# chao1224/GeoSSL

Hardware: AMD Instinct MI355X
Metric: molecules/s/GPU SchNet+DDM fwd+bwd (QM9-sized, bs=1024); % HBM roofline (higher is better)
Workload: dtype f32

## Files before the change

### geossl_amd/Geom3D/models/schnet.py

```python
import ctypes as C
import math
import os

import torch
from ...switches import env as _env
from torch.nn import Embedding, Linear, ModuleList, Sequential

from ... import _lib, ops
from ..._lib import call, ptr, stream
from ...layout import get_layout
from ._atomic_mass import atomic_masses

SUPPORTED_F = (32, 64, 128)


class _Ssp(torch.autograd.Function):
    @staticmethod
    def forward(ctx, x):
        x = x.contiguous()
        y = torch.empty_like(x)
        call("geossl_ssp_fwd", ptr(x), x.numel(), ptr(y), stream())
        ctx.save_for_backward(y)
        return y

# ... 208 lines not shown
        g_emb, g_head = grads[0], grads[1 + 9 * L:]
        g_layers = [grads[1 + 9 * l: 1 + 9 * (l + 1)] for l in range(L)]
        dh_out = dhout.contiguous()
        dyn = getattr(lay, "dyn", None)
        dN2, dP2 = (dyn.n_atoms2, dyn.n_pairs2) if dyn is not None else (None, None)
        probs = []
        daggs = [None] * L
        if cfg["chain"]:
            img = sv.get("img_bwd")
            if img is None:
                img = ops.prepare_chain([lp[k] for lp in layers for k in (4, 5, 7)] + [head[0], head[2]], transB=False)
            i_lin1, i_lin2, i_lin = img[0:3 * L:3], img[1:3 * L:3], img[2:3 * L:3]
            full = lambda: torch.empty(N, F, dtype=torch.float32, device=dev)
            du = full()
            dhs = [full() for _ in range(L + 1)]
            dys, dxs = [full() for _ in range(L)], [full() for _ in range(L)]
            daggs = [full() for _ in range(L)]

            def run_rows(a0, a1, mols, todo=None):
                rows = lambda t_: t_[a0:a1]

                def chain(x_, stages):
                    if todo is not None:
                        todo.append(("chain", x_, stages))
                    else:
                        ops.linear_chain(x_, stages, dyn_rows=dN2)

                chain(rows(dh_out), [dict(image=img[3 * L + 1], tprev=rows(sv["u"]), out=rows(du)),
                                     dict(image=img[3 * L], out=rows(dhs[L]))])
                chain(rows(dhs[L]), [dict(image=i_lin[L - 1], tprev=rows(sv["ts"][L - 1]), out=rows(dys[L - 1])),
                                     dict(image=i_lin2[L - 1], out=rows(daggs[L - 1]))])
                for l in reversed(range(L)):
                    if todo is not None:
                        todo.append(("agg", daggs[l], sv["Wf"][l], dxs[l], True))
                    else:
                        ops.aggregate(daggs[l], sv["Wf"][l], sv["pair_flag"], lay, swap=True, out=dxs[l],
                                      mols=mols)
                    stages = [dict(image=i_lin1[l], res=rows(dhs[l + 1]), out=rows(dhs[l]))]
                    if l > 0:
                        stages += [dict(image=i_lin[l - 1], tprev=rows(sv["ts"][l - 1]), out=rows(dys[l - 1])),
                                   dict(image=i_lin2[l - 1], out=rows(daggs[l - 1]))]
                    chain(rows(dxs[l]), stages)

            todo = [] if (cfg["loop"] and lay.P > 0 and 2 * L + 2 <= _lib.LOOP_MAX_OPS) else None
            if todo is not None:
                run_rows(0, N, None, todo)
                if not ops.layer_loop(todo, lay, sv["pair_flag"], N, F, stagger=cfg["loop_stagger"]):
                    todo = None
            if todo is None:
                run_rows(0, N, None)
            probs.append((dh_out, sv["u"], g_head[2], g_head[3]))
            probs.append((du, sv["h_last"], g_head[0], g_head[1]))
            for l in reversed(range(L)):
                gl = g_layers[l]
                probs.append((dhs[l + 1], sv["ts"][l], gl[7], gl[8]))
                probs.append((dys[l], sv["aggs"][l], gl[5], gl[6]))
                probs.append((dxs[l], sv["hs"][l], gl[4], None))
            dh = dhs[0]
        else:
            du = ops.linear(dh_out, head[2], transB=False, tprev=sv["u"])
            dh = ops.linear(du, head[0], transB=False)
            probs.append((dh_out, sv["u"], g_head[2], g_head[3]))
            probs.append((du, sv["h_last"], g_head[0], g_head[1]))
            pw = ops.prepare_linear([lp[k] for lp in layers for k in (4, 5, 7)], transB=False)
            for l in reversed(range(L)):
                lp, gl = layers[l], g_layers[l]
                w_lin1, w_lin2, w_lin = (pw[3 * l], pw[3 * l + 1], pw[3 * l + 2]) if pw is not None else (lp[4], lp[5], lp[7])
                dy = ops.linear(dh, w_lin, transB=False, tprev=sv["ts"][l])
                dagg = ops.linear(dy, w_lin2, transB=False)
                dx = ops.aggregate(dagg, sv["Wf"][l], sv["pair_flag"], lay, swap=True)
                dh_new = ops.linear(dx, w_lin1, transB=False, res=dh)
                probs.append((dh, sv["ts"][l], gl[7], gl[8]))
                probs.append((dy, sv["aggs"][l], gl[5], gl[6]))
                probs.append((dx, sv["hs"][l], gl[4], None))
                daggs[l] = dagg
                dh = dh_new
        P = lay.P
        fw = _lib.FilterWeights()
        gin = _lib.FilterGradIn()
        for l, lp in enumerate(layers):
            fw.w1[l], fw.b1[l], fw.w2[l], fw.b2[l] = ptr(lp[0]), ptr(lp[1]), ptr(lp[2]), ptr(lp[3])
            gin.x[l], gin.dagg[l] = ptr(sv["xs"][l]), ptr(daggs[l])
        if want_params:
            ops.linear_wgrad(probs, N, F, F, accumulate=bool(accum), dyn_rows=dN2)
            nfl = _lib.load().geossl_embedding_bwd_workspace_floats(emb_w.size(0), F)
            ws = torch.empty(nfl, dtype=torch.float32, device=dev)
            z = ctx.z
            call("geossl_embedding_bwd_dyn", ptr(z), z.stride(0) if z.numel() else 1, ptr(dh), emb_w.size(0), N, F,
                 ptr(g_emb), ptr(ws), accum, dN2, st)
            if P > 0:
                gout = _lib.FilterGradOut()
                for l, gl in enumerate(g_layers):
                    gout.dw1[l], gout.db1[l], gout.dw2[l], gout.db2[l] = ptr(gl[0]), ptr(gl[1]), ptr(gl[2]), ptr(gl[3])
                nfl = _lib.load().geossl_cfconv_filter_bwd_workspace_floats(P, L, F, G)
                ws2 = torch.empty(nfl, dtype=torch.float32, device=dev)
                call("geossl_cfconv_filter_bwd_dyn", ptr(sv["pair_d"]), ptr(sv["pair_c"]), ptr(sv["pair_flag"]),
                     ptr(lay.pair_i), ptr(lay.pair_j), P, N, C.byref(fw), C.byref(gin), L, F, G, ptr(cfg["offset"]),
                     cfg["coeff"], ptr(sv["T"]), C.byref(gout), ptr(ws2), accum, dP2, dN2, st)
            elif not direct:
                for gl in g_layers:
                    for k in range(4):
                        gl[k].zero_()
        dpos = None
        if want_pos:
            dpos = torch.zeros(N, 3, dtype=torch.float32, device=dev)
            if P > 0:
                dd = torch.empty(L, P, dtype=torch.float32, device=dev)
                call("geossl_cfconv_filter_dpos", ptr(sv["pair_d"]), ptr(sv["pair_c"]), ptr(sv["pair_flag"]),
                     ptr(lay.pair_i), ptr(lay.pair_j), P, C.byref(fw), C.byref(gin), L, F, G, ptr(cfg["offset"]),
                     cfg["coeff"], cfg["cutoff"], ptr(sv["T"]), ptr(sv["Wf"]), ptr(dd), st)
                call("geossl_pair_position_grad", ptr(ctx.pos), ptr(sv["pair_d"]), ptr(dd), ptr(lay.mol_ptr),
                     ptr(lay.pair_ptr), lay.B, P, L, ptr(dpos), st)
        if direct:
            return dpos, [None] * len(grads)
        return dpos, list(grads)


class _SchNetTapeCore(torch.autograd.Function):

    @staticmethod
    def forward(ctx, z, pos, lay, cfg, *params):
        from ... import tape as tp
        with torch.no_grad():
            x = tp.leaf(pos, bool(ctx.needs_input_grad[1]))
            ps = [tp.leaf(p, bool(n)) for p, n in zip(params, ctx.needs_input_grad[4:])]
            h = tp.schnet_atom_features(z, x, lay, cfg, ps)
        ctx.tape = (h, x, ps)
        ctx.shapes = [tuple(p.shape) for p in params]
        return h.t

    @staticmethod
    def backward(ctx, dh):
        from ... import tape as tp
        if torch.is_grad_enabled():
            raise NotImplementedError("second-order gradients (training on forces) need the fused widths: "
                                      "hidden_channels == num_filters in %s" % (SUPPORTED_F,))
        h, x, ps = ctx.tape
        wrt = [v for v in [x] + ps if v.req]
        with torch.no_grad():
            got = iter(tp.grad([h], [tp.const(dh.contiguous())], wrt))
        vals = [next(got) if v.req else None for v in [x] + ps]
        dpos = None if vals[0] is None else vals[0].t
        grads = [None if g is None else g.t.reshape(shape) for g, shape in zip(vals[1:], ctx.shapes)]
        return (None, dpos, None, None) + tuple(grads)


class _SegmentReduce(torch.autograd.Function):

    @staticmethod
    def forward(ctx, h, lay, reduce):
        ctx.lay, ctx.reduce = lay, reduce
        return ops.segment_reduce(h.contiguous(), lay, reduce)

    @staticmethod
    def backward(ctx, dout):
        return _SegmentExpand.apply(dout, ctx.lay, ctx.reduce), None, None


class _SegmentExpand(torch.autograd.Function):

    @staticmethod
    def forward(ctx, dout, lay, reduce):
        ctx.lay, ctx.reduce = lay, reduce
        dh = torch.empty(lay.N, dout.size(1), dtype=torch.float32, device=dout.device)
        call("geossl_segment_reduce_bwd", ptr(dout.contiguous()), ptr(lay.mol_ptr), lay.B, dout.size(1),
             1 if reduce == "mean" else 0, ptr(dh), 0, stream())
        return dh

    @staticmethod
    def backward(ctx, g):
        return _SegmentReduce.apply(g, ctx.lay, ctx.reduce), None, None


class SchNet(torch.nn.Module):
    def __init__(self, hidden_channels=128, num_filters=128, num_interactions=6, num_gaussians=50, cutoff=10.0,
                 node_class=None, readout="mean", dipole=False, mean=None, std=None, atomref=None):
        super().__init__()
        assert readout in ["add", "sum", "mean"]
        self.hidden_channels = hidden_channels
        self.num_filters = num_filters
        self.num_interactions = num_interactions
# ... 99 lines not shown
```

### geossl_amd/NCSN.py

```python
import ctypes as C
import os

import numpy as np
import torch
from .switches import env as _env
import torch.nn as nn
import torch.nn.functional as F

from . import _lib
from ._lib import call, ptr, stream
from .layout import get_super_edge_layout


class MultiLayerPerceptron(nn.Module):

    def __init__(self, input_dim, hidden_dims, activation="relu", dropout=0):
        super().__init__()
        self.dims = [input_dim] + hidden_dims
        self.activation = getattr(F, activation) if isinstance(activation, str) else None
        self.dropout = nn.Dropout(dropout) if dropout else None
        self.layers = nn.ModuleList()
        for i in range(len(self.dims) - 1):
            self.layers.append(nn.Linear(self.dims[i], self.dims[i + 1]))
        self.reset_parameters()
# ... 148 lines not shown
        pss = (ps[:npar], ps[npar:])
        dyn = getattr(sel, "dyn", None)
        ctx.dyn = dyn
        if dyn is not None:
            hs = (h1.detach().contiguous(),) * 2
            ctx.grad_slots = (None, None)
        else:
            hs = (h1.detach().contiguous(), h2.detach().contiguous())
            ctx.grad_slots = (getattr(h1, "_geossl_grad_slot", None), getattr(h2, "_geossl_grad_slot", None))
        heads = (_lib.NcsnHeadFwd * 2)()
        keep, saved, ws = [], [], []
        for k, (h, d, nl, dn) in enumerate(((hs[0], d1, nl1, dn1), (hs[1], d2, nl2, dn2))):
            hd = heads[k]
            d, nl, dn = d.contiguous(), nl.contiguous(), dn.contiguous()
            keep += [d, nl, dn]
            for name, p in zip(_FIELDS, pss[k]):
                setattr(hd.w, name, ptr(p))
            hd.w.sigmas = ptr(sigmas[k])
            hd.h, hd.distance, hd.noise_level, hd.distance_noise = ptr(h), ptr(d), ptr(nl), ptr(dn)
            hd.anneal_power = float(powers[k])
            loss_e = torch.empty(S, dtype=torch.float32, device=dev)
            sv = {}
            if training:
                sv = dict(a1=torch.empty(S, Fd, dtype=torch.float32, device=dev),
                          a2=torch.empty(S, Fd // 2, dtype=torch.float32, device=dev),
                          pd=torch.empty(S, dtype=torch.float32, device=dev),
                          emb=torch.empty(S, dtype=torch.float32, device=dev),
                          gscale=torch.empty(S, dtype=torch.float32, device=dev))
                for name in ("a1", "a2", "pd", "emb", "gscale"):
                    setattr(hd.saved, name, ptr(sv[name]))
            w_ = torch.empty(256, dtype=torch.float32, device=dev)
            hd.loss_e, hd.workspace = ptr(loss_e), ptr(w_)
            keep.append(loss_e)
            saved.append(sv)
            ws.append(w_)
        st = stream()
        call("geossl_ddm_loss_fwd2_dyn", C.byref(heads), ptr(sel.batch), ptr(sel.sei0), ptr(sel.sei1), S, Fd,
             None if dyn is None else dyn.n_super, None if dyn is None else dyn.n_atoms, st)
        loss = torch.empty((), dtype=torch.float32, device=dev)
        call("geossl_loss_reduce_partials2", ptr(ws[0]), ptr(ws[1]), ptr(sel.stats), float(out_scale), float(out_scale),
             ptr(loss), st)
        if training:
            ctx.sel, ctx.pss, ctx.saved, ctx.hs, ctx.sigmas = sel, pss, saved, hs, sigmas
            ctx.params, ctx.npar, ctx.out_scale = params, npar, float(out_scale)
        return loss

    @staticmethod
    def backward(ctx, gout):
        sel, pss, saved, hs = ctx.sel, ctx.pss, ctx.saved, ctx.hs
        dev = hs[0].device
        S, Fd, N = sel.S, hs[0].size(1), hs[0].size(0)
        st = stream()
        gout = gout.contiguous().to(torch.float32)
        direct = _lib.direct_grads_enabled(ctx.params)
        grads = [p.grad for p in ctx.params] if direct else [torch.empty_like(p) for p in pss[0] + pss[1]]
        gs = (grads[:ctx.npar], grads[ctx.npar:])
        lib = _lib.load()
        heads = (_lib.NcsnHeadBwd * 2)()
        keep, dhs = [], []
        nws = int(lib.geossl_ddm_loss_bwd_fused_workspace_floats(S, Fd))
        dyn = ctx.dyn
        dh_all = torch.empty(N, Fd, dtype=torch.float32, device=dev) if dyn is not None else None
        for k in range(2):
            hd = heads[k]
            for name, p in zip(_FIELDS, pss[k]):
                setattr(hd.w, name, ptr(p))
            hd.w.sigmas = ptr(ctx.sigmas[k])
            for name in ("a1", "a2", "pd", "emb", "gscale"):
                setattr(hd.saved, name, ptr(saved[k][name]))
            for name, t_ in zip(_FIELDS, gs[k]):
                setattr(hd.grads, name, ptr(t_))
            dfeat = torch.empty(S, Fd, dtype=torch.float32, device=dev)
            demb = torch.empty(S, dtype=torch.float32, device=dev)
            grow = torch.empty(S, dtype=torch.float32, device=dev)
            ws1 = torch.empty(nws, dtype=torch.float32, device=dev)
            slot = ctx.grad_slots[k]
            dh = dh_all if dyn is not None else (slot.rows(N, Fd, torch.float32, dev) if slot is not None else None)
            if dh is None:
                dh = torch.empty(N, Fd, dtype=torch.float32, device=dev)
            hd.h, hd.out_scale, hd.dfeat, hd.demb, hd.grow, hd.workspace, hd.dh = (
                ptr(hs[k]), ctx.out_scale, ptr(dfeat), ptr(demb), ptr(grow), ptr(ws1), ptr(dh))
            keep += [dfeat, demb, grow, ws1]
            dhs.append(dh)
        call("geossl_ddm_loss_bwd_fused2_dyn", C.byref(heads), ptr(sel.sei0), ptr(sel.sei1), S, sel.N if dyn is not None else N,
             Fd, ptr(sel.stats), ptr(gout), ptr(sel.inc_ptr), ptr(sel.inc_idx), 1 if direct else 0,
             None if dyn is None else dyn.n_super, None if dyn is None else dyn.n_atoms, st)
        head = ((dh_all, None) if dyn is not None else (dhs[0], dhs[1])) + (None,) * 11
        if direct:
            return head + (None,) * len(grads)
        return head + tuple(grads)


def ddm_heads_loss(n1, n2, data, h1, distance_1, h2, distance_2, noise_level_1=None, distance_noise_1=None,
                   noise_level_2=None, distance_noise_2=None, out_scale=0.5):
    ok = (isinstance(n1, NCSN_version_03) and isinstance(n2, NCSN_version_03) and n1.emb_dim == n2.emb_dim
          and n1.emb_dim in (32, 64, 128) and not _env("GEOSSL_NCSN_SPLIT_BWD")
          and not _env("GEOSSL_ARITH_24BIT")
          and not _env("GEOSSL_NCSN_SEPARATE_HEADS")
          and (h2 is None or h1.shape == h2.shape) and not distance_1.requires_grad and not distance_2.requires_grad
          and n1 is not n2 and not ({id(p) for p in _head_params(n1)} & {id(p) for p in _head_params(n2)}))
    if ok:
        S_, N_, Fd = data.super_edge_index.size(1), h1.size(0), h1.size(1)
        ok = S_ > 0 and max(S_, N_) * Fd * 4 < 2 ** 32
    bucket = getattr(data, "_bucket", None)
    if bucket is not None and (not ok or h2 is not None):
        raise _lib.GeosslHipError("a capacity-bucket batch needs the paired NCSN heads on one fused feature tensor")
    if not ok:
        return (n1(data, h1, distance_1, noise_level=noise_level_1, distance_noise=distance_noise_1, out_scale=out_scale) +
                n2(data, h2, distance_2, noise_level=noise_level_2, distance_noise=distance_noise_2, out_scale=out_scale))
    _lib.require_cuda(h1, h2, distance_1, distance_2, n1.sigmas, n2.sigmas)
    n1.device = n2.device = n1.sigmas.device
    num_graphs = data.num_graphs
    sel = bucket.sel if bucket is not None else get_super_edge_layout(data.batch, data.super_edge_index, num_graphs)
    draws = []
    for n_, nl, dn, d in ((n1, noise_level_1, distance_noise_1, distance_1), (n2, noise_level_2, distance_noise_2, distance_2)):
        if nl is None:
            nl = torch.randint(0, n_.sigmas.size(0), (num_graphs,), device=n_.sigmas.device)
        if dn is None:
            dn = torch.randn_like(d)
        draws.append((nl, dn))
    p1, p2 = _head_params(n1), _head_params(n2)
    return _NcsnLossPair.apply(h1, h2, distance_1.view(-1), distance_2.view(-1), draws[0][0], draws[0][1].view(-1),
                               draws[1][0], draws[1][1].view(-1), sel, (n1.sigmas.detach(), n2.sigmas.detach()),
                               (n1.anneal_power, n2.anneal_power), out_scale, len(p1), *p1, *p2)


class NCSN_version_03(torch.nn.Module):
    def __init__(self, emb_dim, sigma_begin, sigma_end, num_noise_level, noise_type, anneal_power):
        super().__init__()
        self.anneal_power = anneal_power
        self.noise_type = noise_type
        self.input_distance_mlp = MultiLayerPerceptron(1, [emb_dim, 1], activation="relu")
        self.output_mlp = MultiLayerPerceptron(1 + emb_dim, [emb_dim, emb_dim // 2, 1])
        sigmas = torch.tensor(np.exp(np.linspace(np.log(sigma_begin), np.log(sigma_end), num_noise_level)),
                              dtype=torch.float32)
        self.sigmas = nn.Parameter(sigmas, requires_grad=False)
        self.emb_dim = emb_dim

    def forward(self, data, node_feature, distance, debug=False, noise_level=None, distance_noise=None,
                out_scale=1.0):
        self.device = self.sigmas.device
        _lib.require_cuda(node_feature, distance, self.sigmas)
        if self.emb_dim not in (32, 64, 128):
            raise NotImplementedError("HIP path supports emb_dim in (32, 64, 128)")
        if distance.requires_grad:
            raise NotImplementedError("gradient w.r.t. distance/positions is not built (SURVEY.md §8(f) N3)")
        num_graphs = data.num_graphs
        sel = get_super_edge_layout(data.batch, data.super_edge_index, num_graphs)
        if noise_level is None:
            noise_level = torch.randint(0, self.sigmas.size(0), (num_graphs,), device=self.device)
        if distance_noise is None:
            distance_noise = torch.randn_like(distance)
        if sel.S == 0:
            raise ValueError("batch has no super edges (scatter_add over an empty index fails in the reference too)")
        loss = _NcsnLoss.apply(node_feature, distance.view(-1), noise_level, distance_noise.view(-1), sel,
                               self.sigmas.detach(), self.anneal_power, out_scale, *_head_params(self))
        if debug:
            print("loss", float(loss))
        return loss
```

### geossl_amd/_lib.py

```python
import ctypes as C
import os

import torch

HERE = os.path.dirname(os.path.abspath(__file__))
LIB_PATH = os.path.join(HERE, "lib", "libgeossl_hip.so")

MAX_L = 12
TN_MAX = 32
EPI_BIAS, EPI_SSP, EPI_RESIDUAL, EPI_MUL_DSSP, CHAIN_SAME_INPUT, CHAIN_NEW_INPUT, CHAIN_ADD_PREV = 1, 2, 4, 8, 16, 32, 64
EPI_SILU, EPI_MUL_DSILU = 128, 256

vp = C.c_void_p
i64 = C.c_int64
i32 = C.c_int
f32 = C.c_float
f64 = C.c_double
u64 = C.c_uint64


class FilterWeights(C.Structure):
    _fields_ = [("w1", vp * MAX_L), ("b1", vp * MAX_L), ("w2", vp * MAX_L), ("b2", vp * MAX_L)]


# ... 174 lines not shown
    "geossl_cfconv_filter_fwd_dyn": (i32, [vp, vp, i64, P(FilterWeights), i32, i32, i32, vp, f32, vp, vp, vp, vp]),
    "geossl_cfconv_filter_bwd_dyn": (i32, [vp, vp, vp, vp, vp, i64, i64, P(FilterWeights), P(FilterGradIn), i32, i32, i32,
                                           vp, f32, vp, P(FilterGradOut), vp, i32, vp, vp, vp]),
    "geossl_cfconv_aggregate_work_dyn": (i32, [vp, vp, vp, vp, vp, vp, i64, i32, i32, i32, vp, vp, vp]),
    "geossl_cfconv_aggregate_targets_dyn": (i32, [vp, vp, vp, vp, vp, vp, i64, i32, i32, i32, vp, vp, vp]),
    "geossl_linear_chain_dyn": (i32, [vp, i32, P(Chain), i64, i32, vp, vp]),
    "geossl_linear_wgrad_dyn": (i32, [P(TnBatch), i32, i64, i32, i32, i32, i32, i32, vp, i32, vp, vp]),
    "geossl_ddm_loss_fwd2_dyn": (i32, [vp, vp, vp, vp, i64, i32, vp, vp, vp]),
    "geossl_ddm_loss_bwd_fused2_dyn": (i32, [vp, vp, vp, i64, i64, i32, vp, vp, vp, vp, i32, vp, vp, vp]),
    "geossl_painn_group_capacity": (i64, [i64, i64]),
    "geossl_painn_edge_layout": (i32, [vp, vp, i64, vp, i64, i64, i64] + [vp] * 12),
    "geossl_painn_edge_geom_dyn": (i32, [vp, vp, vp, i64, f32, vp, vp, i32, vp, vp, vp, vp, vp]),
    "geossl_painn_interaction_fwd_mma_dyn": (i32, [vp, vp, vp, vp, vp, vp, vp, vp, vp, vp, vp, vp, vp, i64, i32, i64, i32,
                                                   i32, vp, vp, vp, vp]),
    "geossl_tape_unary": (i32, [i32, vp, i64, f32, f32, vp, vp]),
    "geossl_tape_binary": (i32, [i32, vp, i32, vp, i32, i64, i32, f32, vp, vp]),
    "geossl_tape_colsum_workspace_floats": (i64, [i64, i32]),
    "geossl_tape_reduce": (i32, [i32, vp, i64, i32, vp, vp, vp]),
    "geossl_tape_gather_rows": (i32, [vp, vp, i32, i64, i32, vp, vp]),
    "geossl_tape_scatter_rows": (i32, [vp, vp, i32, vp, i64, i32, vp, vp]),
    "geossl_tape_copy2d": (i32, [vp, i64, vp, i64, i64, i32, vp]),
    "geossl_tape_fill": (i32, [vp, i64, f32, vp]),
    "geossl_painn_stage_cap": (i32, [i32, i32, i32]),
    "geossl_painn_interaction_fwd_atoms": (i32, [vp] * 12 + [i64, vp, i32, i32, vp, vp, vp]),
    "geossl_painn_interaction_bwd_atoms": (i32, [vp] * 13 + [i64, vp, i32, i32, vp, vp, vp, vp, vp, i32, vp]),
    "geossl_painn_interaction_bwd_mol_skip": (i32, [vp, vp, vp, vp, vp, vp, vp, vp, vp, vp, vp, vp, vp, i64, i32, i64, i32,
                                                    i32, vp, vp, vp, vp, vp, i32, vp]),
    "geossl_painn_mix_pre_fwd_dyn": (i32, [vp, vp, i64, i32, f32, vp, vp, vp, vp]),
    "geossl_painn_mix_post_fwd_dyn": (i32, [vp, vp, vp, vp, vp, i64, i32, vp, vp, vp, vp]),
    "geossl_painn_mix_post_bwd_dyn": (i32, [vp, vp, vp, vp, vp, i64, i32, vp, vp, vp, vp]),
    "geossl_painn_mix_pre_bwd_dyn": (i32, [vp, vp, vp, vp, i64, i32, vp, vp, vp, vp]),
    "geossl_gather_molecules": (i32, [P(Gather), i64, vp]),
    "geossl_gather_masked_molecules": (i32, [P(Gather), P(Mask), i64, vp]),
    "geossl_infonce_fwd": (i32, [vp, vp, i64, i32, f32, vp, vp, vp, vp, vp]),
    "geossl_infonce_bwd": (i32, [vp, vp, vp, vp, i64, i32, f32, vp, vp, vp, vp]),
    "geossl_ebm_nce_fwd": (i32, [vp, vp, i64, i32, i32, vp, vp, vp, vp, vp, vp]),
    "geossl_ebm_nce_bwd": (i32, [vp, vp, vp, i64, i32, i32, vp, vp, vp, vp]),
    "geossl_distance_head_width_ok": (i32, [i32]),
    "geossl_distance_head_fwd_workspace_floats": (i64, [i64]),
    "geossl_distance_head_bwd_workspace_floats": (i64, [i64, i32]),
    "geossl_distance_head_fwd": (i32, [vp, i64, i32, vp, vp, vp, vp, vp, i64, vp, vp, vp, vp, vp, vp]),
    "geossl_distance_head_fwd_dyn": (i32, [vp, i64, i32, vp, vp, vp, vp, vp, i64, vp, vp, vp, vp, vp, vp, vp, vp]),
    "geossl_distance_head_bwd": (i32, [vp, i64, i32, vp, vp, i64, vp, vp, vp, vp, vp, vp, vp, vp, i32, vp]),
    "geossl_distance_head_bwd_dyn": (i32, [vp, i64, i32, vp, vp, i64, vp, vp, vp, vp, vp, vp, vp, vp, i32, vp, vp, vp]),
    "geossl_charge_mask_count": (i64, [i64, f64]),
    "geossl_charge_mask": (i32, [vp, i32, i64, f64, i32, vp, vp, vp, vp, vp, vp]),
    "geossl_charge_mask_dyn": (i32, [vp, i32, i64, f64, i32, vp, vp, vp, vp, vp, vp, vp]),
    "geossl_charge_head_width_ok": (i32, [i32, i32]),
    "geossl_charge_head_fwd_workspace_floats": (i64, [i64]),
    "geossl_charge_head_bwd_workspace_floats": (i64, [i64, i32, i32]),
    "geossl_charge_head_fwd": (i32, [vp, i64, i32, vp, vp, i32, vp, vp, i64, vp, vp, vp, vp, vp, vp]),
    "geossl_charge_head_fwd_dyn": (i32, [vp, i64, i32, vp, vp, i32, vp, vp, i64, vp, vp, vp, vp, vp, vp, vp]),
    "geossl_charge_head_bwd": (i32, [vp, i64, i32, vp, i32, vp, vp, i64, vp, vp, vp, vp, vp, vp, vp, i32, vp]),
    "geossl_charge_head_bwd_dyn": (i32, [vp, i64, i32, vp, i32, vp, vp, i64, vp, vp, vp, vp, vp, vp, vp, i32, vp, vp]),
    "geossl_infograph_width_ok": (i32, [i32]),
    "geossl_infograph_fwd_workspace_floats": (i64, [i64]),
    "geossl_infograph_fwd": (i32, [vp, i64, i32, vp, vp, i64, i32, vp, vp, vp, vp, vp, vp, vp, vp]),
    "geossl_infograph_fwd_dyn": (i32, [vp, i64, i32, vp, vp, i64, i32, vp, vp, vp, vp, vp, vp, vp, vp, vp]),
    "geossl_infograph_bwd": (i32, [vp, i64, i32, vp, vp, i64, i32, vp, vp, vp, vp, vp, vp, vp, vp]),
    "geossl_infograph_bwd_dyn": (i32, [vp, i64, i32, vp, vp, i64, i32, vp, vp, vp, vp, vp, vp, vp, vp, vp]),
    "geossl_property_width_ok": (i32, [i32]),
    "geossl_property_workspace_floats": (i64, [i64]),
    "geossl_property_fwd": (i32, [vp, i64, i32, vp, i64, i32, i32, vp, vp, vp, vp, vp, i64, vp, i32, vp, vp, vp, vp, vp,
                                  vp]),
    "geossl_property_fwd_dyn": (i32, [vp, i64, i32, vp, i64, i32, i32, vp, vp, vp, vp, vp, i64, vp, i32, vp, vp, vp, vp,
                                      vp, vp, vp]),
    "geossl_property_predict": (i32, [vp, i64, i32, vp, i64, i32, i32, vp, vp, vp, vp, vp, vp, vp]),
    "geossl_property_predict_dyn": (i32, [vp, i64, i32, vp, i64, i32, i32, vp, vp, vp, vp, vp, vp, vp, vp]),
    "geossl_property_bwd": (i32, [i64, i32, vp, i64, i32, i32, vp, vp, vp, vp, vp, vp, i64, vp, i32, vp, vp, vp, vp, vp,
                                  vp, i32, vp]),
    "geossl_property_bwd_dyn": (i32, [i64, i32, vp, i64, i32, i32, vp, vp, vp, vp, vp, vp, i64, vp, i32, vp, vp, vp, vp,
                                      vp, vp, i32, vp, vp]),
    "geossl_property_targets": (i32, [vp, i64, i32, i32, vp, vp, i64, vp, vp]),
    "geossl_torsion_head_width_ok": (i32, [i32]),
    "geossl_torsion_head_fwd_workspace_floats": (i64, [i64]),
    "geossl_torsion_head_bwd_workspace_floats": (i64, [i64, i32]),
    "geossl_torsion_head_fwd": (i32, [vp, i64, i32, vp, vp, vp, vp, vp, vp, i64, vp, vp, vp, vp, vp, vp]),
    "geossl_torsion_head_fwd_dyn": (i32, [vp, i64, i32, vp, vp, vp, vp, vp, vp, i64, vp, vp, vp, vp, vp, vp, vp, vp]),
    "geossl_torsion_head_bwd": (i32, [vp, i64, i32, vp, vp, vp, vp, i64, vp, vp, i64, vp, vp, vp, vp, vp, i32, vp]),
    "geossl_torsion_head_bwd_dyn": (i32, [vp, i64, i32, vp, vp, vp, vp, i64, vp, vp, i64, vp, vp, vp, vp, vp, i32, vp, vp,
                                          vp]),
    "geossl_triple_angles": (i32, [vp, i64, vp, vp, vp, i64, vp, vp]),
    "geossl_gather_triples": (i32, [vp, i64, vp, vp, vp, vp, i64, vp, vp, vp, vp, vp]),
}

_lib = None


class GeosslHipError(RuntimeError):
    pass


def load():
    global _lib
    if _lib is not None:
        return _lib
    path = os.environ.get("GEOSSL_HIP_LIB", LIB_PATH)
    if not os.path.exists(path):
        raise GeosslHipError(
            "libgeossl_hip.so is not built (%s). Run `python -m geossl_amd.build` (needs hipcc); "
            "there is no CPU fallback." % path)
    lib = C.CDLL(path)
    for name, (res, args) in PROTOTYPES.items():
        fn = getattr(lib, name)
        fn.restype = res
        fn.argtypes = args
    if lib.geossl_abi_version() != 1:
        raise GeosslHipError("ABI version mismatch")
    _lib = lib
    return lib


def check(rc, what):
    if rc != 0:
        raise GeosslHipError("%s failed with hipError %d" % (what, rc))


def ptr(t):
    if t is None:
        return None
    return t.data_ptr()


def stream():
    return torch._C._cuda_getCurrentRawStream(torch._C._cuda_getDevice())


def require_cuda(*tensors):
    for t in tensors:
        if t is not None and not t.is_cuda:
            raise GeosslHipError(
                "geossl_amd runs on MI355X only: got a %s tensor. The HIP path has no CPU fallback." % t.device.type)



_DIRECT = {"depth": 0}


class direct_grads:
    def __enter__(self):
        _DIRECT["depth"] += 1
        return self

    def __exit__(self, *exc):
        _DIRECT["depth"] -= 1
        return False


def direct_grads_enabled(params):
    return _DIRECT["depth"] > 0 and all(
        p.grad is not None and p.grad.is_contiguous() and p.grad.dtype == torch.float32 and p.grad.is_cuda
        for p in params)


class StatusWord:

    def __init__(self, device, message):
        self.word = torch.zeros(1, dtype=torch.int32, device=device)
        self.host = torch.zeros(1, dtype=torch.int32).pin_memory()
        self.event = None
        self.message = message

    def __deepcopy__(self, memo):
        return None

    def __reduce__(self):
        return (type(None), ())

    def poll(self):
        if self.event is None or torch.cuda.is_current_stream_capturing():
            return
        if self.event.query():
            self.event = None
            if int(self.host[0]):
                raise IndexError(self.message)

    def arm(self, every=1):
        self.calls = getattr(self, "calls", 0) + 1
        if every > 1 and self.calls % every != 1:
            return
        if self.event is None and not torch.cuda.is_current_stream_capturing():
            self.host.copy_(self.word, non_blocking=True)
            self.event = torch.cuda.Event()
            self.event.record()

    def check(self):
        if int(self.word.item()):
            raise IndexError(self.message)


def module_status(module, device, message):
    st = module.__dict__.get("_geossl_status")
    if st is None or st.word.device != device:
        st = StatusWord(device, message)
        module.__dict__["_geossl_status"] = st
    return st


TIMERS = None
CALLS = None


def call(name, *args):
    global CALLS
    lib = load()
    if CALLS is not None:
        CALLS += 1
    timers = TIMERS
    key = name[:-4] if name.endswith("_dyn") else name
    if timers is not None and key in timers:
        e0, e1 = torch.cuda.Event(enable_timing=True), torch.cuda.Event(enable_timing=True)
        e0.record()
        rc = getattr(lib, name)(*args)
        e1.record()
        timers[key].append((e0, e1))
    else:
        rc = getattr(lib, name)(*args)
    check(rc, name)


def fill_ptrs(arr, tensors):
    for i, t in enumerate(tensors):
        arr[i] = ptr(t)
```

### geossl_amd/build.py

```python
import os
import subprocess
import sys

HERE = os.path.dirname(os.path.abspath(__file__))
REPO = os.path.dirname(HERE)
CSRC = os.path.join(HERE, "csrc")
LIB_DIR = os.path.join(HERE, "lib")
LIB_PATH = os.path.join(LIB_DIR, "libgeossl_hip.so")


def _sources():
    return sorted(f for f in os.listdir(CSRC) if f.endswith(".hip"))


SOURCE_FLAGS = {"painn_mma.hip": ["-fno-slp-vectorize"], "distance_head.hip": ["-fno-slp-vectorize"],
                "charge_head.hip": ["-fno-slp-vectorize"], "infograph_head.hip": ["-fno-slp-vectorize"],
                "property_head.hip": ["-fno-slp-vectorize"], "torsion_head.hip": ["-fno-slp-vectorize"]}


def _headers():
    hs = [os.path.join(CSRC, f) for f in os.listdir(CSRC) if f.endswith(".h")]
    inc = os.path.join(REPO, "include")
    return hs + [os.path.join(inc, f) for f in os.listdir(inc) if f.endswith(".h")]


def source_hash():
    import hashlib
    h = hashlib.sha256()
    h.update(repr(sorted(SOURCE_FLAGS.items())).encode())
    for path in sorted([os.path.join(CSRC, s_) for s_ in _sources()] + _headers()):
        h.update(os.path.basename(path).encode() + b"\0")
        with open(path, "rb") as fh:
            h.update(fh.read())
    return h.hexdigest()[:16]


def _newest(paths):
    return max(os.path.getmtime(p) for p in paths)


def needs_build():
    if not os.path.exists(LIB_PATH):
        return True
    deps = [os.path.join(CSRC, s) for s in _sources()] + _headers() + [os.path.abspath(__file__)]
    return _newest(deps) > os.path.getmtime(LIB_PATH)


def build(force=False, verbose=True):
    if not force and not needs_build():
        return LIB_PATH
    os.makedirs(LIB_DIR, exist_ok=True)
    hipcc = os.environ.get("HIPCC", "/opt/rocm/bin/hipcc")
    objs = []
    procs = []
    for s in _sources():
        obj = os.path.join(LIB_DIR, s.replace(".hip", ".o"))
        cmd = [hipcc, "--offload-arch=gfx950", "-O3", "-std=c++17", "-fPIC", "-I", os.path.join(REPO, "include"),
               "-I", CSRC, "-Wno-pass-failed"] + SOURCE_FLAGS.get(s, []) + ["-c", os.path.join(CSRC, s), "-o", obj]
        if verbose:
            print(" ".join(cmd), flush=True)
        procs.append((cmd, subprocess.Popen(cmd)))
        objs.append(obj)
    for cmd, p in procs:
        if p.wait() != 0:
            raise RuntimeError("hipcc failed: " + " ".join(cmd))
    cmd = [hipcc, "--offload-arch=gfx950", "-shared", "-fPIC", "-o", LIB_PATH] + objs
    if verbose:
        print(" ".join(cmd), flush=True)
    subprocess.check_call(cmd)
    return LIB_PATH


if __name__ == "__main__":
    build(force="--force" in sys.argv)
    print(LIB_PATH)
```

### geossl_amd/csrc/common.h

```cpp
#pragma once
#include <hip/hip_runtime.h>
#include <stdint.h>

#include <mutex>

typedef float f32x16 __attribute__((ext_vector_type(16)));
typedef float f32x4 __attribute__((ext_vector_type(4)));

#define GEOSSL_MAX_LAYERS 12
#define GEOSSL_PI_F 3.14159265358979323846f

#define GEOSSL_CHECK_LAUNCH()                  \
  do {                                         \
    hipError_t e__ = hipGetLastError();        \
    if (e__ != hipSuccess) return (int)e__;    \
  } while (0)

namespace geossl {

inline void allow_big_lds_ptr(const void* kernel) {
  struct Seen { const void* fn; int dev; };
  static Seen seen[512];
  static int nseen = 0;
  static std::mutex mu;
// ... 21 lines not shown
#pragma clang fp contract(off)
  const float xx = x * x, yy = y * y, zz = z * z;
  return (xx + yy) + zz;
}

__device__ __forceinline__ void lds_barrier() {
  asm volatile("s_waitcnt lgkmcnt(0)\n\ts_barrier" ::: "memory");
}

__device__ __forceinline__ float wave_max(float v) {
  v = fmaxf(v, __builtin_bit_cast(float, __builtin_amdgcn_update_dpp(0, __builtin_bit_cast(int, v), 0xB1, 0xF, 0xF, false)));
  v = fmaxf(v, __builtin_bit_cast(float, __builtin_amdgcn_update_dpp(0, __builtin_bit_cast(int, v), 0x4E, 0xF, 0xF, false)));
  v = fmaxf(v, __builtin_bit_cast(float, __builtin_amdgcn_update_dpp(0, __builtin_bit_cast(int, v), 0x141, 0xF, 0xF, false)));
  v = fmaxf(v, __builtin_bit_cast(float, __builtin_amdgcn_update_dpp(0, __builtin_bit_cast(int, v), 0x140, 0xF, 0xF, false)));
  const float a = __builtin_bit_cast(float, __builtin_amdgcn_readlane(__builtin_bit_cast(int, v), 0));
  const float b = __builtin_bit_cast(float, __builtin_amdgcn_readlane(__builtin_bit_cast(int, v), 16));
  const float c = __builtin_bit_cast(float, __builtin_amdgcn_readlane(__builtin_bit_cast(int, v), 32));
  const float d = __builtin_bit_cast(float, __builtin_amdgcn_readlane(__builtin_bit_cast(int, v), 48));
  return fmaxf(fmaxf(a, b), fmaxf(c, d));
}
__device__ __forceinline__ int wave_max_i32(int v) {
  v = max(v, __builtin_amdgcn_update_dpp(v, v, 0xB1, 0xF, 0xF, false));
  v = max(v, __builtin_amdgcn_update_dpp(v, v, 0x4E, 0xF, 0xF, false));
  v = max(v, __builtin_amdgcn_update_dpp(v, v, 0x141, 0xF, 0xF, false));
  v = max(v, __builtin_amdgcn_update_dpp(v, v, 0x140, 0xF, 0xF, false));
  return max(max(__builtin_amdgcn_readlane(v, 0), __builtin_amdgcn_readlane(v, 16)),
             max(__builtin_amdgcn_readlane(v, 32), __builtin_amdgcn_readlane(v, 48)));
}
__device__ __forceinline__ int c_row(int reg, int lane) { return (reg & 3) + 8 * (reg >> 2) + 4 * (lane >> 5); }

#define GEOSSL_SSP_SHIFT 0.693147182464599609375f
__device__ __forceinline__ float exp_neg(float x) { return __builtin_amdgcn_exp2f(x * 1.44269504088896340736f); }
__device__ __forceinline__ float ssp(float x) {
  const float z = exp_neg(-fabsf(x));
  const float l = __builtin_amdgcn_logf(1.0f + z);
  return fmaf(l, 0.693147180559945309417f, fmaxf(x, 0.0f)) - GEOSSL_SSP_SHIFT;
}
__device__ __forceinline__ float dssp_from_out(float t) { return 1.0f - 0.5f * exp_neg(-t); }

template <class ValFn, class ConsumeFn>
__device__ __forceinline__ void transpose_c_block(float* stage, int lane, ValFn val, ConsumeFn consume) {
  const int j = lane & 31, kh = lane >> 5;
  const int rr = lane >> 3, c4 = lane & 7;
#pragma unroll
  for (int half = 0; half < 2; ++half) {
#pragma unroll
    for (int q = 0; q < 8; ++q) {
      const int r = 8 * half + q;
      const int row16 = (r & 3) + 8 * ((r >> 2) & 1) + 4 * kh;
      stage[row16 * 32 + j] = val(r);
    }
    asm volatile("s_waitcnt lgkmcnt(0)" ::: "memory");
#pragma unroll
    for (int u = 0; u < 2; ++u) {
      const int row16 = 8 * u + rr;
      const float4 v = *reinterpret_cast<const float4*>(stage + row16 * 32 + 4 * c4);
      consume(16 * half + row16, 4 * c4, v);
    }
    asm volatile("s_waitcnt lgkmcnt(0)" ::: "memory");
  }
}

__device__ __forceinline__ float pin(float v) {
  asm volatile("" : "+v"(v));
  return v;
}
__device__ __forceinline__ float4 pin(float4 v) {
  asm volatile("" : "+v"(v.x), "+v"(v.y), "+v"(v.z), "+v"(v.w));
  return v;
}

__device__ __forceinline__ float kahan_sum_strided(const float* __restrict__ p, int b0, int b1, int stride) {
#pragma clang fp reassociate(off) contract(off)
  float s = 0.0f, c = 0.0f;
#pragma unroll 4
  for (int b = b0; b < b1; ++b) {
    const float y = p[(size_t)b * stride] - c;
    const float t = s + y;
    c = (t - s) - y;
    s = t;
  }
  return s;
}

__device__ __forceinline__ int dyn_count(int cap, const int32_t* __restrict__ dyn) {
  return dyn != nullptr ? min(cap, *dyn) : cap;
}

__device__ __forceinline__ float wave_sum(float v) {
#pragma unroll
  for (int o = 32; o > 0; o >>= 1) v += __shfl_xor(v, o, 64);
  return v;
}

}
```

### geossl_amd/csrc/filter_bwd.hip

```cpp
#include "common.h"
#include "geossl_hip.h"
#include "split.h"
#include "tn.h"

using namespace geossl;

namespace {

#ifdef FB_TIMING
__device__ long long fb_dbg[2 * 64 * 8];
__device__ long long fb_dbg2[2 * 64];
__device__ long long fb_dbg3[64 * 4];
#define FB_MARK(slot)                                                                                   \
  do {                                                                                                  \
    if (blockIdx.x == 3 && blockIdx.y == 0 && lane == 0 && (wave == 0 || wave == NW) && t - t_begin < 64) \
      fb_dbg[((wave == 0 ? 0 : 1) * 64 + (t - t_begin)) * 8 + (slot)] = clock64();                      \
  } while (0)
#define FB3(slot)                                                                                      \
  do {                                                                                                  \
    __builtin_amdgcn_sched_barrier(0);                                                                  \
    if (blockIdx.x == 3 && blockIdx.y == 0 && lane == 0 && wave == NW && tt - t_begin < 64 && tt > t_begin) \
      fb_dbg3[(tt - t_begin) * 4 + (slot)] = clock64();                                                  \
    __builtin_amdgcn_sched_barrier(0);                                                                  \
  } while (0)
// ... 1043 lines not shown

}

#ifdef FB_TIMING
extern "C" int geossl_filter_bwd_debug_read(long long* host) {
  return (int)hipMemcpyFromSymbol(host, HIP_SYMBOL(fb_dbg), sizeof(long long) * 2 * 64 * 8);
}
extern "C" int geossl_filter_bwd_debug_read3(long long* host) {
  return (int)hipMemcpyFromSymbol(host, HIP_SYMBOL(fb_dbg3), sizeof(long long) * 64 * 4);
}
extern "C" int geossl_filter_bwd_debug_read2(long long* host) {
  return (int)hipMemcpyFromSymbol(host, HIP_SYMBOL(fb_dbg2), sizeof(long long) * 2 * 64);
}
#endif

extern "C" int64_t geossl_cfconv_filter_bwd_workspace_floats(int64_t P, int L, int F, int G) {
  const int ntiles = (int)((P + TR - 1) / TR);
  const int64_t nb = blocks_per_layer(L, ntiles);
  return (int64_t)L * nb * ((int64_t)F * G + F + (int64_t)F * F + F);
}

extern "C" int geossl_cfconv_filter_bwd(const float* pair_d, const float* pair_c, const uint8_t* pair_flag,
                                        const int32_t* pair_i, const int32_t* pair_j, int64_t P, int64_t N,
                                        const GeosslFilterWeights* w, const GeosslFilterGradIn* g, int L, int F, int G,
                                        const float* offset, float coeff, const float* T,
                                        const GeosslFilterGradOut* out, float* workspace, int accumulate,
                                        hipStream_t stream) {
  return geossl_cfconv_filter_bwd_dyn(pair_d, pair_c, pair_flag, pair_i, pair_j, P, N, w, g, L, F, G, offset, coeff, T, out,
                                      workspace, accumulate, nullptr, nullptr, stream);
}

extern "C" int geossl_cfconv_filter_bwd_dyn(const float* pair_d, const float* pair_c, const uint8_t* pair_flag,
                                            const int32_t* pair_i, const int32_t* pair_j, int64_t P, int64_t N,
                                            const GeosslFilterWeights* w, const GeosslFilterGradIn* g, int L, int F,
                                            int G, const float* offset, float coeff, const float* T,
                                            const GeosslFilterGradOut* out, float* workspace, int accumulate,
                                            const int32_t* dyn_P, const int32_t* dyn_N, hipStream_t stream) {
  if (P <= 0 || L <= 0) return 0;
  if (L > GEOSSL_MAX_L || (F != 32 && F != 64 && F != 128) || G > 64) return (int)hipErrorInvalidValue;
  const int ntiles = (int)((P + TR - 1) / TR);
  const int nb = blocks_per_layer(L, ntiles);
  dim3 grid(nb, L);
  float* pw1 = workspace;
  float* pb1 = pw1 + (size_t)L * nb * F * G;
  float* pw2 = pb1 + (size_t)L * nb * F;
  float* pb2 = pw2 + (size_t)L * nb * F * F;
#define LAUNCH(NW)                                                                                                 \
  do {                                                                                                             \
    const size_t lds = BwdLds<32 * NW>::bytes();                                                                   \
    allow_big_lds(&k_filter_bwd<NW>);                                                                              \
    hipLaunchKernelGGL((k_filter_bwd<NW>), grid, dim3(128 * NW), lds, stream, pair_d, pair_c, pair_flag, pair_i,   \
                       pair_j, (int)P, (int)N, *w, *g, G, offset, coeff, T, pw1, pb1, pw2, pb2, dyn_P, dyn_N);     \
  } while (0)
#define LAUNCH_H(NW)                                                                                               \
  do {                                                                                                             \
    const size_t lds = BwdLdsH<32 * NW>::bytes();                                                                  \
    if (T == nullptr) {                                                                                            \
      allow_big_lds(&k_filter_bwd_h<NW, true>);                                                                    \
      hipLaunchKernelGGL((k_filter_bwd_h<NW, true>), grid, dim3(128 * NW), lds, stream, pair_d, pair_c, pair_flag, \
                         pair_i, pair_j, (int)P, (int)N, *w, *g, G, offset, coeff, T, pw1, pb1, pw2, pb2, dyn_P,   \
                         dyn_N);                                                                                   \
    } else {                                                                                                       \
      allow_big_lds(&k_filter_bwd_h<NW, false>);                                                                   \
      hipLaunchKernelGGL((k_filter_bwd_h<NW, false>), grid, dim3(128 * NW), lds, stream, pair_d, pair_c, pair_flag,\
                         pair_i, pair_j, (int)P, (int)N, *w, *g, G, offset, coeff, T, pw1, pb1, pw2, pb2, dyn_P,   \
                         dyn_N);                                                                                   \
    }                                                                                                              \
  } while (0)
  const bool bf16x3 = getenv("GEOSSL_FILTER_BWD_BF16X3") != nullptr || getenv("GEOSSL_ARITH_24BIT") != nullptr;
  if (bf16x3 && T == nullptr) return (int)hipErrorInvalidValue;
  if (!bf16x3) {
    if (F == 128) LAUNCH_H(4); else if (F == 64) LAUNCH_H(2); else LAUNCH_H(1);
  } else {
    if (F == 128) LAUNCH(4); else if (F == 64) LAUNCH(2); else LAUNCH(1);
  }
#undef LAUNCH_H
#undef LAUNCH
  GEOSSL_CHECK_LAUNCH();
  ReduceMulti rm;
  rm.add(pw1, F * G, G, G, 1, out->dw1, L);
  rm.add(pb1, F, F, F, 1, out->db1, L);
  rm.add(pw2, F * F, F, F, 1, out->dw2, L);
  rm.add(pb2, F, F, F, 1, out->db2, L);
  hipLaunchKernelGGL(k_reduce_multi, dim3(rm.blocks(), L), dim3(256), 0, stream, rm, nb, accumulate);
  GEOSSL_CHECK_LAUNCH();
  return 0;
}
```

### geossl_amd/csrc/ncsn_bwd.hip

```cpp
#include "common.h"
#include "geossl_hip.h"
#include "split.h"
#include "tn.h"

using namespace geossl;

namespace {

constexpr int TR = 32;

#ifdef NB_TIMING
__device__ long long nb_dbg[2 * 32 * 8];
#define NB_MARK(slot)                                                                              \
  do {                                                                                             \
    if (blockIdx.x == 5 && lane == 0 && (wave == 0 || wave == NW) && t - t_begin < 32)             \
      nb_dbg[((wave == 0 ? 0 : 1) * 32 + (t - t_begin)) * 8 + (slot)] = clock64();                 \
  } while (0)
#else
#define NB_MARK(slot) do {} while (0)
#endif

template <int NW>
struct NbLds {
  static constexpr int F = 32 * NW, H = F / 2, KHS = (H + 15) / 16, HMB = (H + 31) / 32, KS = F / 16;
  u32x4* zb;
  u32x4* dz2T;
  u32x4* fT;
  u32x4* dz1r;
  u32x4* abT;
  int4* scal;
  float* pdv;
  float* dep;
  float* wls;
  int* eg;
  int* ef;
  int* ea;
  int* ec;
  __device__ explicit NbLds(uint8_t* smem) {
    zb = reinterpret_cast<u32x4*>(smem);
    dz2T = zb + 2 * KHS * 2 * 64;
    fT = dz2T + HMB * 2 * 2 * 64;
    dz1r = fT + 2 * NW * 2 * 2 * 64;
    abT = dz1r + KS * 2 * 64;
    scal = reinterpret_cast<int4*>(abT + NW * 2 * 2 * 64);
    pdv = reinterpret_cast<float*>(scal + 3 * TR);
    dep = pdv + 3 * TR;
    wls = dep + NW * TR;
    eg = reinterpret_cast<int*>(wls + F);
    ef = eg + 4;
    ea = ef + 2 * NW;
    ec = ea + NW;
  }
  static size_t bytes() {
    return (size_t)(2 * KHS * 2 + HMB * 4 + 2 * NW * 4 + KS * 2 + NW * 4) * 1024 + 3 * TR * sizeof(int4) +
           (size_t)(3 * TR + NW * TR + F) * sizeof(float) + (size_t)(4 + 4 * NW) * sizeof(int);
  }
};

struct NcsnFusedArgs {
  const float* h;
  const int64_t* sei0;
  const int64_t* sei1;
  int S;
  GeosslNcsnWeights w;
  GeosslNcsnSaved sv;
  const int64_t* divisor;
  float out_scale;
  const float* gout;
  float* dfeat;
  float* demb;
  float* grow;
  float* pw1;
  float* pd1;
  float* pb1;
  float* pw2;
  float* pb2;
  float* psm;
};

__device__ __forceinline__ float ldg_off(const float* base, uint32_t byte_off) {
  return *reinterpret_cast<const float*>(reinterpret_cast<const char*>(base) + byte_off);
}
__device__ __forceinline__ int crow4(int r, int k4) { return (r & 3) + 8 * (r >> 2) + k4; }
__device__ __forceinline__ int opaque(int v) {
  asm volatile("" : "+v"(v));
  return v;
// ... 473 lines not shown
    }
    NB_MARK(4);
  }
  const size_t pb = blockIdx.x;
  if constexpr (ROLE_A) {
    float* P1 = a.pw1 + pb * F * F;
#pragma unroll
    for (int kb = 0; kb < NW; ++kb) {
      const float f = pow2(max(E1[kb] + eC - 28, -200));
#pragma unroll
      for (int r = 0; r < 16; ++r) P1[(size_t)(32 * nb + c_row(r, lane)) * F + 32 * kb + j] = accw1[kb][r] * f;
    }
    const float sb = bsum + __shfl_xor(bsum, 32, 64), sd = dsum + __shfl_xor(dsum, 32, 64);
    if (kh == 0) {
      a.pb1[pb * F + col] = sb;
      a.pd1[pb * F + col] = sd;
    }
    float* Ps = a.psm + pb * (H + 3 * F + 2);
    const float t_w2 = s_w2 + __shfl_xor(s_w2, 32, 64);
    const float t_w1 = s_w1 + __shfl_xor(s_w1, 32, 64), t_b1 = s_b1 + __shfl_xor(s_b1, 32, 64);
    if (kh == 0) {
      Ps[H + col] = t_w2;
      Ps[H + F + col] = t_w1;
      Ps[H + 2 * F + col] = t_b1;
    }
    if (wave == 0) {
      const float tg = wave_sum(s_g), td = wave_sum(s_d);
      if (lane == 0) {
        Ps[H + 3 * F] = tg;
        Ps[H + 3 * F + 1] = td;
      }
    }
  } else {
    float* P2 = a.pw2 + pb * H * F;
    const float f = pow2(max(E2 + e3 - 28, -200));
#pragma unroll
    for (int mb = 0; mb < HMB; ++mb)
#pragma unroll
      for (int r = 0; r < 16; ++r) {
        const int m = 32 * mb + c_row(r, lane);
        if (m < H) P2[(size_t)m * F + col] = accw2[mb][r] * f;
      }
    const float sb = bsum + __shfl_xor(bsum, 32, 64);
    if (nb < HMB && kh == 0 && (int)col < H) a.pb2[pb * H + col] = sb;
    if (nb < KHS) {
      float* Ps = a.psm + pb * (H + 3 * F + 2);
#pragma unroll
      for (int e = 0; e < 8; ++e) {
        float v = o3acc[e];
#pragma unroll
        for (int o = 16; o > 0; o >>= 1) v += __shfl_xor(v, o, 64);
        const int m = 16 * nb + 8 * kh + e;
        if (j == 0 && m < H) Ps[m] = v;
      }
    }
  }
}

template <int NW>
__global__ __launch_bounds__(128 * NW) void k_ncsn_bwd_fused(NcsnFusedArgs a) {
  if ((int)(threadIdx.x >> 6) < NW) ncsn_bwd_body<NW, true>(a, a.S, a.h);
  else ncsn_bwd_body<NW, false>(a, a.S, a.h);
}
struct NcsnFusedPair { NcsnFusedArgs a[2]; };
template <int NW>
__global__ __launch_bounds__(128 * NW) void k_ncsn_bwd_fused2(NcsnFusedPair pr, const int32_t* __restrict__ dyn_S,
                                                              const int32_t* __restrict__ dyn_view) {
  const NcsnFusedArgs& a = pr.a[blockIdx.y];
  const int S = dyn_count(a.S, dyn_S);
  const float* h = a.h;
  if (dyn_view != nullptr && blockIdx.y == 1) h += (size_t)(*dyn_view) * (32 * NW);
  if ((int)(threadIdx.x >> 6) < NW) ncsn_bwd_body<NW, true>(a, S, h);
  else ncsn_bwd_body<NW, false>(a, S, h);
}

__device__ __forceinline__ void ncsn_reduce_all_block(const ReduceMulti& m, int nblk, int accumulate,
                                                      const float* __restrict__ psm, int F, const GeosslNcsnGrads& g,
                                                      float (*red)[64]) {
  const int mb = m.xoff[m.nseg];
  if ((int)blockIdx.x < mb) {
    reduce_multi_block(m, nblk, accumulate, red, 0);
    return;
  }
  const int H = F / 2, len = H + 3 * F + 2;
  const int i = ((int)blockIdx.x - mb) * 4 + (int)(threadIdx.x >> 6), lane = threadIdx.x & 63;
  if (i >= len) return;
  float s = 0.0f;
  for (int b = lane; b < nblk; b += 64) s += psm[(size_t)b * len + i];
  s = wave_sum(s);
  if (lane == 0) {
    float* dst;
    if (i < H) dst = g.o3_w + i;
    else if (i < H + F) dst = g.in_w2 + (i - H);
    else if (i < H + 2 * F) dst = g.in_w1 + (i - H - F);
    else if (i < H + 3 * F) dst = g.in_b1 + (i - H - 2 * F);
    else if (i == H + 3 * F) dst = g.o3_b;
    else dst = g.in_b2;
    *dst = accumulate ? *dst + s : s;
  }
}
__global__ __launch_bounds__(256) void k_ncsn_reduce_all(ReduceMulti m, int nblk, int accumulate,
                                                         const float* __restrict__ psm, int F, GeosslNcsnGrads g) {
  __shared__ float red[4][64];
  ncsn_reduce_all_block(m, nblk, accumulate, psm, F, g, red);
}
__global__ __launch_bounds__(256) void k_ncsn_reduce_all2(ReduceMulti m0, ReduceMulti m1, int nblk, int accumulate,
                                                          const float* __restrict__ psm0,
                                                          const float* __restrict__ psm1, int F, GeosslNcsnGrads g0,
                                                          GeosslNcsnGrads g1) {
  __shared__ float red[4][64];
  if (blockIdx.y == 0) ncsn_reduce_all_block(m0, nblk, accumulate, psm0, F, g0, red);
  else ncsn_reduce_all_block(m1, nblk, accumulate, psm1, F, g1, red);
}

inline int fused_blocks(int64_t S) {
  const int64_t ntiles = (S + TR - 1) / TR;
  return (int)(ntiles < 256 ? ntiles : 256);
}

}

#ifdef NB_TIMING
extern "C" int geossl_ncsn_bwd_debug_read(long long* host) {
  return (int)hipMemcpyFromSymbol(host, HIP_SYMBOL(nb_dbg), sizeof(long long) * 2 * 32 * 8);
}
#endif

extern "C" int64_t geossl_ddm_loss_bwd_fused_workspace_floats(int64_t S, int F) {
  const int64_t nb = fused_blocks(S), H = F / 2;
  return nb * ((int64_t)F * F + 2 * F + H * F + H + (H + 3 * F + 2));
}

extern "C" int geossl_ddm_loss_bwd_fused(const float* h, const int64_t* sei0, const int64_t* sei1, int64_t S, int64_t N,
                                         int F, const GeosslNcsnWeights* w, const GeosslNcsnSaved* saved,
                                         const int64_t* stats_divisor, float out_scale, const float* gout, float* dfeat,
                                         float* demb, float* grow, const GeosslNcsnGrads* grads, float* workspace,
                                         int accumulate, hipStream_t stream) {
  if (S <= 0) return 0;
  if (F != 32 && F != 64 && F != 128) return (int)hipErrorInvalidValue;
  if (S * (int64_t)F * 4 >= ((int64_t)1 << 32) || N * (int64_t)F * 4 >= ((int64_t)1 << 32)) return (int)hipErrorInvalidValue;
  const int nb = fused_blocks(S), H = F / 2;
  NcsnFusedArgs a;
  a.h = h; a.sei0 = sei0; a.sei1 = sei1; a.S = (int)S; a.w = *w; a.sv = *saved; a.divisor = stats_divisor;
  a.out_scale = out_scale; a.gout = gout; a.dfeat = dfeat; a.demb = demb; a.grow = grow;
  a.pw1 = workspace;
  a.pd1 = a.pw1 + (size_t)nb * F * F;
  a.pb1 = a.pd1 + (size_t)nb * F;
  a.pw2 = a.pb1 + (size_t)nb * F;
  a.pb2 = a.pw2 + (size_t)nb * H * F;
  a.psm = a.pb2 + (size_t)nb * H;
#define LAUNCH(NWV)                                                                                      \
  do {                                                                                                   \
    allow_big_lds(&k_ncsn_bwd_fused<NWV>);                                                               \
    hipLaunchKernelGGL((k_ncsn_bwd_fused<NWV>), dim3(nb), dim3(128 * NWV), NbLds<NWV>::bytes(), stream, a); \
  } while (0)
  if (F == 128) LAUNCH(4); else if (F == 64) LAUNCH(2); else LAUNCH(1);
#undef LAUNCH
  GEOSSL_CHECK_LAUNCH();
  ReduceMulti rm;
  float* o1w[1] = {grads->o1_w};
  float* o1c[1] = {grads->o1_w + F};
  float* o1b[1] = {grads->o1_b};
  float* o2w[1] = {grads->o2_w};
  float* o2b[1] = {grads->o2_b};
  rm.add(a.pw1, F * F, F, F + 1, 1, o1w, 1);
  rm.add(a.pd1, F, F, F, F + 1, o1c, 1);
  rm.add(a.pb1, F, F, F, 1, o1b, 1);
  rm.add(a.pw2, H * F, F, F, 1, o2w, 1);
  rm.add(a.pb2, H, H, H, 1, o2b, 1);
  hipLaunchKernelGGL(k_ncsn_reduce_all, dim3(rm.blocks() + (H + 3 * F + 2 + 3) / 4, 1), dim3(256), 0, stream, rm, nb,
                     accumulate, a.psm, F, *grads);
  GEOSSL_CHECK_LAUNCH();
  return 0;
}

namespace geossl {
int launch_incidence_gather2(const float* dfeat0, const float* dfeat1, const int64_t* inc_ptr, const int32_t* inc_idx,
                             int64_t N, int F, float* dh0, float* dh1, hipStream_t stream, const int32_t* dyn_view);
}

extern "C" int geossl_ddm_loss_bwd_fused2(const GeosslNcsnHeadBwd* heads, const int64_t* sei0, const int64_t* sei1,
                                          int64_t S, int64_t N, int F, const int64_t* stats_divisor, const float* gout,
                                          const int64_t* inc_ptr, const int32_t* inc_idx, int accumulate,
                                          hipStream_t stream) {
  return geossl_ddm_loss_bwd_fused2_dyn(heads, sei0, sei1, S, N, F, stats_divisor, gout, inc_ptr, inc_idx, accumulate,
                                        nullptr, nullptr, stream);
}

extern "C" int geossl_ddm_loss_bwd_fused2_dyn(const GeosslNcsnHeadBwd* heads, const int64_t* sei0, const int64_t* sei1,
                                              int64_t S, int64_t N, int F, const int64_t* stats_divisor,
                                              const float* gout, const int64_t* inc_ptr, const int32_t* inc_idx,
                                              int accumulate, const int32_t* dyn_S, const int32_t* dyn_view,
                                              hipStream_t stream) {
  if (S <= 0) return 0;
  if (heads == nullptr || (F != 32 && F != 64 && F != 128)) return (int)hipErrorInvalidValue;
  if (S * (int64_t)F * 4 >= ((int64_t)1 << 32) || N * (int64_t)F * 4 >= ((int64_t)1 << 32)) return (int)hipErrorInvalidValue;
  const int nb = (fused_blocks(S) + 1) / 2, H = F / 2;
  NcsnFusedPair pr;
  NcsnFusedArgs* a = pr.a;
  for (int k = 0; k < 2; ++k) {
    const GeosslNcsnHeadBwd& hd = heads[k];
    if (hd.h == nullptr || hd.dfeat == nullptr || hd.workspace == nullptr) return (int)hipErrorInvalidValue;
    NcsnFusedArgs& x = a[k];
    x.h = hd.h; x.sei0 = sei0; x.sei1 = sei1; x.S = (int)S; x.w = hd.w; x.sv = hd.saved; x.divisor = stats_divisor;
    x.out_scale = hd.out_scale; x.gout = gout; x.dfeat = hd.dfeat; x.demb = hd.demb; x.grow = hd.grow;
    x.pw1 = hd.workspace;
    x.pd1 = x.pw1 + (size_t)nb * F * F;
    x.pb1 = x.pd1 + (size_t)nb * F;
    x.pw2 = x.pb1 + (size_t)nb * F;
    x.pb2 = x.pw2 + (size_t)nb * H * F;
    x.psm = x.pb2 + (size_t)nb * H;
  }
#define LAUNCH2(NWV)                                                                                                \
  do {                                                                                                              \
    allow_big_lds(&k_ncsn_bwd_fused2<NWV>);                                                                         \
    hipLaunchKernelGGL((k_ncsn_bwd_fused2<NWV>), dim3(nb, 2), dim3(128 * NWV), NbLds<NWV>::bytes(), stream, pr,         \
                       dyn_S, dyn_view);                                                                            \
  } while (0)
  if (F == 128) LAUNCH2(4); else if (F == 64) LAUNCH2(2); else LAUNCH2(1);
#undef LAUNCH2
  GEOSSL_CHECK_LAUNCH();
  ReduceMulti rm[2];
  for (int k = 0; k < 2; ++k) {
    const GeosslNcsnGrads* grads = &heads[k].grads;
    float* o1w[1] = {grads->o1_w};
    float* o1c[1] = {grads->o1_w + F};
    float* o1b[1] = {grads->o1_b};
    float* o2w[1] = {grads->o2_w};
    float* o2b[1] = {grads->o2_b};
    rm[k].add(a[k].pw1, F * F, F, F + 1, 1, o1w, 1);
    rm[k].add(a[k].pd1, F, F, F, F + 1, o1c, 1);
    rm[k].add(a[k].pb1, F, F, F, 1, o1b, 1);
    rm[k].add(a[k].pw2, H * F, F, F, 1, o2w, 1);
    rm[k].add(a[k].pb2, H, H, H, 1, o2b, 1);
  }
  hipLaunchKernelGGL(k_ncsn_reduce_all2, dim3(rm[0].blocks() + (H + 3 * F + 2 + 3) / 4, 2), dim3(256), 0, stream, rm[0],
                     rm[1], nb, accumulate, a[0].psm, a[1].psm, F, heads[0].grads, heads[1].grads);
  GEOSSL_CHECK_LAUNCH();
  if (heads[0].dh != nullptr && heads[1].dh != nullptr)
    return launch_incidence_gather2(heads[0].dfeat, heads[1].dfeat, inc_ptr, inc_idx, N, F, heads[0].dh, heads[1].dh, stream,
                                    dyn_view);
  return 0;
}
```

### geossl_amd/csrc/schnet.hip

```cpp
#include "common.h"
#include "aggregate_reg.h"
#include "geossl_hip.h"
#include "tn.h"

#include <cstdlib>

using namespace geossl;

namespace {

inline int grid1d(int64_t n, int block, int cap = 2048) {
  int64_t g = (n + block - 1) / block;
  return (int)(g < 1 ? 1 : (g > cap ? cap : g));
}

__global__ void k_rbf(const float* __restrict__ d, int64_t E, const float* __restrict__ offset, int G, float coeff,
                      float* __restrict__ out) {
  for (int64_t i = (int64_t)blockIdx.x * blockDim.x + threadIdx.x; i < E * G; i += (int64_t)gridDim.x * blockDim.x) {
    const int64_t e = i / G;
    const int g = (int)(i - e * G);
    const float diff = d[e] - offset[g];
    out[i] = expf(coeff * (diff * diff));
  }
}

__global__ void k_ssp_fwd(const float* __restrict__ x, int64_t n, float* __restrict__ y) {
  for (int64_t i = (int64_t)blockIdx.x * blockDim.x + threadIdx.x; i < n; i += (int64_t)gridDim.x * blockDim.x)
    y[i] = ssp(x[i]);
}
__global__ void k_ssp_bwd(const float* __restrict__ y, const float* __restrict__ dy, int64_t n, float* __restrict__ dx) {
  for (int64_t i = (int64_t)blockIdx.x * blockDim.x + threadIdx.x; i < n; i += (int64_t)gridDim.x * blockDim.x)
    dx[i] = dy[i] * dssp_from_out(y[i]);
}

__global__ void k_pair_product(const float* __restrict__ a, const float* __restrict__ b,
                               const int32_t* __restrict__ pair_i, const int32_t* __restrict__ pair_j,
                               const uint8_t* __restrict__ pair_flag, int64_t P, int F, int swap,
                               float* __restrict__ out) {
  const int Q = F / 4;
  for (int64_t idx = (int64_t)blockIdx.x * blockDim.x + threadIdx.x; idx < P * Q; idx += (int64_t)gridDim.x * blockDim.x) {
    const int64_t p = idx / Q;
    const int c = 4 * (int)(idx - p * Q);
    unsigned fl = pair_flag[p];
    if (swap) fl = ((fl & 1u) << 1) | ((fl >> 1) & 1u);
    const float f0 = (fl & 1u) ? 1.0f : 0.0f, f1 = (fl & 2u) ? 1.0f : 0.0f;
    const size_t oi = (size_t)pair_i[p] * F + c, oj = (size_t)pair_j[p] * F + c;
    const f32x4 ai = *reinterpret_cast<const f32x4*>(a + oi), aj = *reinterpret_cast<const f32x4*>(a + oj);
    const f32x4 bi = *reinterpret_cast<const f32x4*>(b + oi), bj = *reinterpret_cast<const f32x4*>(b + oj);
    *reinterpret_cast<f32x4*>(out + (size_t)p * F + c) = f0 * (ai * bj) + f1 * (aj * bi);
  }
}


template <int VW>
struct AggVec;
template <>
struct AggVec<1> {
  typedef float type;
};
template <>
struct AggVec<2> {
  typedef f32x2 type;
};

template <int VW>
__global__ __launch_bounds__(64) void k_aggregate(const float* __restrict__ x, const float* __restrict__ Wf,
                                                  const uint8_t* __restrict__ pair_flag,
                                                  const int32_t* __restrict__ mol_ptr,
                                                  const int32_t* __restrict__ pair_ptr,
                                                  const int32_t* __restrict__ order, int B, int F, int max_n, int swap,
                                                  float* __restrict__ out) {
#pragma clang fp contract(off)
  typedef typename AggVec<VW>::type V;
  extern __shared__ __attribute__((aligned(16))) float smem[];
  if ((int)blockIdx.x >= B) return;
  const int m = order != nullptr ? order[blockIdx.x] : (int)blockIdx.x;
  const int lane = threadIdx.x, f = VW * lane;
  const bool col = f < F;
  const int a0 = mol_ptr[m], n = mol_ptr[m + 1] - a0, base = pair_ptr[m], np = n * (n - 1) / 2;
  float* xs = smem;
  float* acc = smem + max_n * F;
  uint8_t* sfl = reinterpret_cast<uint8_t*>(smem + 2 * max_n * F);
  for (int p = lane; p < np; p += 64) {
    unsigned fl = pair_flag[base + p];
    if (swap) fl = ((fl & 1u) << 1) | ((fl >> 1) & 1u);
    sfl[p] = (uint8_t)fl;
// ... 136 lines not shown
      else if (part == 2) AGG_PART(4, 2); else AGG_PART(4, 3);
    }
  }
#undef AGG_PART
}

__device__ __forceinline__ int work_item(const int32_t* __restrict__ work, int nwork, const int32_t* __restrict__ dyn_nwork) {
  const int nw = dyn_count(nwork, dyn_nwork), b = (int)blockIdx.x;
  if (b >= nw) return -1;
  return work[(b & 7) * (nw >> 3) + (b >> 3)];
}

__global__ __launch_bounds__(64, 2) void k_aggregate_reg_work(
    const float* __restrict__ x, const float* __restrict__ Wf, const uint8_t* __restrict__ pair_flag,
    const int32_t* __restrict__ mol_ptr, const int32_t* __restrict__ pair_ptr, const int32_t* __restrict__ work,
    int nwork, int F, int swap, float* __restrict__ out, const int32_t* __restrict__ dyn_nwork) {
  const int wk = work_item(work, nwork, dyn_nwork);
  if (wk == -1) return;
  const int m = wk & 0x00FFFFFF, part = __builtin_amdgcn_readfirstlane((wk >> 24) & 255);
  const int lane = threadIdx.x, f = 2 * lane < F ? 2 * lane : -2;
  const int a0 = mol_ptr[m], n = mol_ptr[m + 1] - a0, base = pair_ptr[m];
  const int nu = __builtin_amdgcn_readfirstlane(n);
  if (nu > 33) {
    aggregate_targets(x, Wf, pair_flag, a0, n, base, lane, f, F, swap, out, part, part + 1);
    return;
  }
  const int kparts = nu < AGG_K2_MIN ? 1 : (nu < AGG_K4_MIN ? 2 : 4);
#define AGG_CLASS(NM) if (nu <= NM) { aggregate_reg_body<NM>(x, Wf, pair_flag, a0, n, base, lane, f, F, swap, out); return; }
#define AGG_CLASS_BIG(NM) if (nu <= NM) { aggregate_big<NM>(x, Wf, pair_flag, a0, n, base, lane, f, F, swap, out, kparts, part); return; }
  AGG_CLASS(8) AGG_CLASS(12) AGG_CLASS(16) AGG_CLASS(18) AGG_CLASS(20)
  AGG_CLASS_BIG(22) AGG_CLASS_BIG(24) AGG_CLASS_BIG(26) AGG_CLASS_BIG(28) AGG_CLASS_BIG(30) AGG_CLASS_BIG(33)
#undef AGG_CLASS
#undef AGG_CLASS_BIG
}

__global__ __launch_bounds__(64, 2) void k_aggregate_targets(
    const float* __restrict__ x, const float* __restrict__ Wf, const uint8_t* __restrict__ pair_flag,
    const int32_t* __restrict__ mol_ptr, const int32_t* __restrict__ pair_ptr, const int32_t* __restrict__ work,
    int nwork, int F, int swap, float* __restrict__ out, const int32_t* __restrict__ dyn_nwork) {
  const int wk = work_item(work, nwork, dyn_nwork);
  if (wk == -1) return;
  const int m = wk & 0x00FFFFFF, a = __builtin_amdgcn_readfirstlane((wk >> 24) & 255);
  const int lane = threadIdx.x, f = 2 * lane < F ? 2 * lane : -2;
  const int a0 = mol_ptr[m], n = mol_ptr[m + 1] - a0, base = pair_ptr[m];
  aggregate_targets(x, Wf, pair_flag, a0, n, base, lane, f, F, swap, out, a, a + 1);
}

__global__ void k_embedding_fwd(const int64_t* __restrict__ z, int64_t zs, const float* __restrict__ table, int C,
                                int64_t N, int F, float* __restrict__ out, int32_t* __restrict__ status,
                                const int32_t* __restrict__ dyn_N) {
  N = dyn_count((int)N, dyn_N);
  for (int64_t i = (int64_t)blockIdx.x * blockDim.x + threadIdx.x; i < N * F; i += (int64_t)gridDim.x * blockDim.x) {
    const int64_t a = i / F;
    const int f = (int)(i - a * F);
    const int64_t c = z[a * zs];
    if (c < 0 || c >= C) {
      if (status != nullptr) *status = 1;
      out[i] = 0.0f;
    } else {
      out[i] = table[c * F + f];
    }
  }
}
template <int SH4>
__global__ __launch_bounds__(256) void k_embedding_fwd4(const int64_t* __restrict__ z, int64_t zs,
                                                        const float* __restrict__ table, int C, int N,
                                                        float* __restrict__ out, int32_t* __restrict__ status,
                                                        const int32_t* __restrict__ dyn_N) {
  N = dyn_count(N, dyn_N);
  const uint32_t total = (uint32_t)N << SH4;
  for (uint32_t i = blockIdx.x * 256u + threadIdx.x; i < total; i += gridDim.x * 256u) {
    const uint32_t a = i >> SH4, f4 = i & ((1u << SH4) - 1u);
    const int64_t c = z[(int64_t)a * zs];
    f32x4 v = {0.0f, 0.0f, 0.0f, 0.0f};
    if (c < 0 || c >= C) {
      if (status != nullptr) *status = 1;
    } else {
      v = reinterpret_cast<const f32x4*>(table)[((uint32_t)c << SH4) + f4];
    }
    reinterpret_cast<f32x4*>(out)[i] = v;
  }
}

#define GEOSSL_EMB_CHUNKS 512
template <int NG>
__global__ void k_embedding_bwd_partial(const int64_t* __restrict__ z, int64_t zs, const float* __restrict__ dh,
                                        int64_t N, int F, int C, float* __restrict__ partial, int2* __restrict__ band,
                                        const int32_t* __restrict__ dyn_N) {
  extern __shared__ __attribute__((aligned(16))) float smem[];
  N = dyn_count((int)N, dyn_N);
  const int TF = blockDim.x / NG;
  const int chunk = blockIdx.x, grp = threadIdx.x / TF, f = threadIdx.x - grp * TF;
  const int64_t per = (N + (int64_t)gridDim.x - 1) / (int64_t)gridDim.x;
  const int64_t lo = chunk * per, hi = min((int64_t)N, lo + per);
  float* tab = smem + (size_t)grp * C * F;
  int2* gband = reinterpret_cast<int2*>(smem + (size_t)NG * C * F);
  int cmin = C, cmax = -1;
  if (f < F) {
    for (int c = 0; c < C; ++c) tab[c * F + f] = 0.0f;
    constexpr int U = 16;
    for (int64_t a0 = lo + grp; a0 < hi; a0 += (int64_t)U * NG) {
      float v[U];
      int cls[U];
#pragma unroll
      for (int u = 0; u < U; ++u) {
        const int64_t a = min(a0 + (int64_t)u * NG, hi - 1);
        v[u] = dh[a * F + f];
        cls[u] = (int)z[a * zs];
      }
#pragma unroll
      for (int u = 0; u < U; ++u)
        if (a0 + (int64_t)u * NG < hi && cls[u] >= 0 && cls[u] < C) {
          tab[cls[u] * F + f] += v[u];
          cmin = min(cmin, cls[u]);
          cmax = max(cmax, cls[u]);
        }
    }
    if (f == 0) gband[grp] = make_int2(cmin, cmax);
  }
  if (NG > 1) {
    __syncthreads();
    if (grp != 0) return;
    for (int g = 0; g < NG; ++g) {
      cmin = min(cmin, gband[g].x);
      cmax = max(cmax, gband[g].y);
    }
  }
  if (f >= F) return;
  for (int c = cmin; c <= cmax; ++c) {
    float sum = smem[c * F + f];
    for (int g = 1; g < NG; ++g) sum += smem[((size_t)g * C + c) * F + f];
    partial[((size_t)chunk * C + c) * F + f] = sum;
  }
  if (f == 0) band[chunk] = make_int2(cmin, cmax);
}
__global__ __launch_bounds__(256) void k_embedding_bwd_reduce(const float* __restrict__ partial,
                                                              const int2* __restrict__ band, int nchunks, int C, int F,
                                                              float* __restrict__ dtable, int accumulate) {
  constexpr int PERMAX = GEOSSL_EMB_CHUNKS / 4;
  static_assert(PERMAX == 128, "two chunks per lane");
  const int PER = nchunks / 4;
  __shared__ float red[4][64];
  __shared__ int hits[4][PERMAX];
  const int c = blockIdx.y, lane = threadIdx.x & 63, slice = threadIdx.x >> 6;
  const int f = blockIdx.x * 64 + lane;
  int n = 0;
#pragma unroll
  for (int h = 0; h < 2; ++h) {
    const int b = slice * PER + 64 * h + lane;
    const int2 r = 64 * h + lane < PER ? band[b] : make_int2(1, 0);
    const bool hit = c >= r.x && c <= r.y;
    const unsigned long long m = __ballot(hit);
    if (hit) hits[slice][n + __popcll(m & ((1ull << lane) - 1ull))] = b;
    n += __popcll(m);
  }
  __builtin_amdgcn_wave_barrier();
  float s = 0.0f;
  if (f < F) {
#pragma clang fp reassociate(off) contract(off)
    float k = 0.0f;
    const float* p = partial + (size_t)c * F + f;
#pragma unroll 4
    for (int i = 0; i < n; ++i) {
      const float y = p[(size_t)hits[slice][i] * C * F] - k;
      const float t = s + y;
      k = (t - s) - y;
      s = t;
    }
  }
  red[slice][lane] = s;
  __syncthreads();
  if (slice == 0 && f < F) {
    float v = accumulate ? dtable[(size_t)c * F + f] : 0.0f;
    v += red[0][lane];
    v += red[1][lane];
    v += red[2][lane];
    v += red[3][lane];
    dtable[(size_t)c * F + f] = v;
  }
}
__global__ void k_segment_reduce_fwd(const float* __restrict__ h, const int32_t* __restrict__ mol_ptr, int B, int F,
                                     int mean, float* __restrict__ out) {
  const int m = blockIdx.x;
  if (m >= B) return;
  const int a0 = mol_ptr[m], a1 = mol_ptr[m + 1];
  for (int f = threadIdx.x; f < F; f += blockDim.x) {
    float s = 0.0f;
    for (int a = a0; a < a1; ++a) s += h[(size_t)a * F + f];
    if (mean) s = s / fmaxf((float)(a1 - a0), 1.0f);
    out[(size_t)m * F + f] = s;
  }
}
__global__ void k_segment_reduce_bwd(const float* __restrict__ dout, const int32_t* __restrict__ mol_ptr, int B, int F,
                                     int mean, float* __restrict__ dh, int accumulate) {
  const int m = blockIdx.x;
  if (m >= B) return;
  const int a0 = mol_ptr[m], a1 = mol_ptr[m + 1];
  const float cnt = fmaxf((float)(a1 - a0), 1.0f);
  for (int f = threadIdx.x; f < F; f += blockDim.x) {
    float gv = dout[(size_t)m * F + f];
    if (mean) gv = gv / cnt;
    for (int a = a0; a < a1; ++a) {
      const size_t o = (size_t)a * F + f;
      dh[o] = accumulate ? dh[o] + gv : gv;
    }
  }
}

__global__ __launch_bounds__(256) void k_row_normalize_fwd(const float* __restrict__ h, int64_t N, int F, float eps,
                                                           float* __restrict__ y, float* __restrict__ norm) {
  const int lane = threadIdx.x & 63;
  const int64_t row = (int64_t)blockIdx.x * 4 + (threadIdx.x >> 6);
  if (row >= N) return;
  const float* hr = h + row * F;
  float ss = 0.0f;
  for (int f = lane; f < F; f += 64) ss = fmaf(hr[f], hr[f], ss);
  ss = wave_sum(ss);
  const float nr = sqrtf(ss), den = fmaxf(nr, eps);
  for (int f = lane; f < F; f += 64) y[row * F + f] = hr[f] / den;
  if (lane == 0 && norm != nullptr) norm[row] = nr;
}
__global__ __launch_bounds__(256) void k_row_normalize_bwd(const float* __restrict__ g, const float* __restrict__ y,
                                                           const float* __restrict__ norm, int64_t N, int F, float eps,
                                                           float* __restrict__ dh) {
  const int lane = threadIdx.x & 63;
  const int64_t row = (int64_t)blockIdx.x * 4 + (threadIdx.x >> 6);
  if (row >= N) return;
  const float* gr = g + row * F;
  const float* yr = y + row * F;
  float dot = 0.0f;
  for (int f = lane; f < F; f += 64) dot = fmaf(gr[f], yr[f], dot);
  dot = wave_sum(dot);
  const float nr = norm[row];
  const bool clamped = nr < eps;
  const float inv = 1.0f / fmaxf(nr, eps);
  for (int f = lane; f < F; f += 64) dh[row * F + f] = (clamped ? gr[f] : gr[f] - yr[f] * dot) * inv;
}

inline int blocks_per_layer(int L, int ntiles) {
  int b = 256 / (L > 0 ? L : 1);
  if (b < 1) b = 1;
  if (b > ntiles) b = ntiles;
  return b;
}

}

extern "C" int geossl_rbf_fwd(const float* d, int64_t E, const float* offset, int G, float coeff, float* out,
                              hipStream_t stream) {
  if (E <= 0) return 0;
  hipLaunchKernelGGL(k_rbf, dim3(grid1d(E * G, 256)), dim3(256), 0, stream, d, E, offset, G, coeff, out);
  GEOSSL_CHECK_LAUNCH();
  return 0;
}

extern "C" int geossl_ssp_fwd(const float* x, int64_t n, float* y, hipStream_t stream) {
  if (n <= 0) return 0;
  hipLaunchKernelGGL(k_ssp_fwd, dim3(grid1d(n, 256)), dim3(256), 0, stream, x, n, y);
  GEOSSL_CHECK_LAUNCH();
  return 0;
}
extern "C" int geossl_ssp_bwd(const float* y, const float* dy, int64_t n, float* dx, hipStream_t stream) {
// ... 77 lines not shown
    allow_big_lds(&k_aggregate<2>);
    hipLaunchKernelGGL(k_aggregate<2>, dim3((unsigned)B), dim3(64), lds, stream, x, Wf, pair_flag, mol_ptr, pair_ptr,
                       order, (int)B, F, max_n, swap, out);
  } else {
    allow_big_lds(&k_aggregate<1>);
    hipLaunchKernelGGL(k_aggregate<1>, dim3((unsigned)B), dim3(64), lds, stream, x, Wf, pair_flag, mol_ptr, pair_ptr,
                       order, (int)B, F, max_n, swap, out);
  }
  GEOSSL_CHECK_LAUNCH();
  return 0;
}

extern "C" int geossl_row_normalize_fwd(const float* h, int64_t N, int F, float eps, float* y, float* norm,
                                        hipStream_t stream) {
  if (N <= 0) return 0;
  hipLaunchKernelGGL(k_row_normalize_fwd, dim3((unsigned)((N + 3) / 4)), dim3(256), 0, stream, h, N, F, eps, y, norm);
  GEOSSL_CHECK_LAUNCH();
  return 0;
}
extern "C" int geossl_row_normalize_bwd(const float* g, const float* y, const float* norm, int64_t N, int F, float eps,
                                        float* dh, hipStream_t stream) {
  if (N <= 0) return 0;
  hipLaunchKernelGGL(k_row_normalize_bwd, dim3((unsigned)((N + 3) / 4)), dim3(256), 0, stream, g, y, norm, N, F, eps,
                     dh);
  GEOSSL_CHECK_LAUNCH();
  return 0;
}

extern "C" int geossl_embedding_fwd_dyn(const int64_t* z, int64_t z_stride, const float* table, int num_classes,
                                        int64_t N, int F, float* out, int32_t* status, const int32_t* dyn_N,
                                        hipStream_t stream) {
  if (N <= 0) return 0;
  if (N > 0x7FFFFFFF) return (int)hipErrorInvalidValue;
  const bool al16 = ((reinterpret_cast<uintptr_t>(table) | reinterpret_cast<uintptr_t>(out)) & 15) == 0;
  if (al16 && (F == 32 || F == 64 || F == 128) && N * (F / 4) < ((int64_t)1 << 31)) {
    const dim3 grid(grid1d(N * (F / 4), 256)), block(256);
    if (F == 128) hipLaunchKernelGGL(k_embedding_fwd4<5>, grid, block, 0, stream, z, z_stride, table, num_classes, (int)N, out, status, dyn_N);
    else if (F == 64) hipLaunchKernelGGL(k_embedding_fwd4<4>, grid, block, 0, stream, z, z_stride, table, num_classes, (int)N, out, status, dyn_N);
    else hipLaunchKernelGGL(k_embedding_fwd4<3>, grid, block, 0, stream, z, z_stride, table, num_classes, (int)N, out, status, dyn_N);
    GEOSSL_CHECK_LAUNCH();
    return 0;
  }
  hipLaunchKernelGGL(k_embedding_fwd, dim3(grid1d(N * F, 256)), dim3(256), 0, stream, z, z_stride, table, num_classes, N,
                     F, out, status, dyn_N);
  GEOSSL_CHECK_LAUNCH();
  return 0;
}

extern "C" int geossl_embedding_fwd(const int64_t* z, int64_t z_stride, const float* table, int num_classes, int64_t N,
                                    int F, float* out, int32_t* status, hipStream_t stream) {
  return geossl_embedding_fwd_dyn(z, z_stride, table, num_classes, N, F, out, status, nullptr, stream);
}

extern "C" int64_t geossl_embedding_bwd_workspace_floats(int num_classes, int F) {
  return (int64_t)GEOSSL_EMB_CHUNKS * num_classes * F + 2 * GEOSSL_EMB_CHUNKS;
}

extern "C" int geossl_embedding_bwd(const int64_t* z, int64_t z_stride, const float* dh, int num_classes, int64_t N,
                                    int F, float* dtable, float* workspace, int accumulate, hipStream_t stream) {
  return geossl_embedding_bwd_dyn(z, z_stride, dh, num_classes, N, F, dtable, workspace, accumulate, nullptr, stream);
}

extern "C" int geossl_embedding_bwd_dyn(const int64_t* z, int64_t z_stride, const float* dh, int num_classes, int64_t N,
                                        int F, float* dtable, float* workspace, int accumulate, const int32_t* dyn_N,
                                        hipStream_t stream) {
  if (num_classes <= 0) return 0;
  if (N > 0x7FFFFFFF) return (int)hipErrorInvalidValue;
  if (F > 256 || (size_t)num_classes * F * sizeof(float) > 160 * 1024) return (int)hipErrorInvalidValue;
  int2* band = reinterpret_cast<int2*>(workspace + (size_t)GEOSSL_EMB_CHUNKS * num_classes * F);
  const int TF = (F + 63) / 64 * 64;
  const int ng = ((size_t)4 * num_classes * F * sizeof(float) <= 48 * 1024 && 4 * TF <= 1024) ? 4 : 1;
  int nchunks = (int)((N + 32 * ng - 1) / (32 * ng));
  nchunks = nchunks < 16 ? 16 : (nchunks > GEOSSL_EMB_CHUNKS ? GEOSSL_EMB_CHUNKS : (nchunks + 3) / 4 * 4);
  const size_t lds = (size_t)ng * num_classes * F * sizeof(float) + ng * sizeof(int2);
  if (ng == 4) {
    hipLaunchKernelGGL(k_embedding_bwd_partial<4>, dim3(nchunks), dim3(4 * TF), lds, stream, z, z_stride, dh, N, F,
                       num_classes, workspace, band, dyn_N);
  } else {
    allow_big_lds(&k_embedding_bwd_partial<1>);
    hipLaunchKernelGGL(k_embedding_bwd_partial<1>, dim3(nchunks), dim3(TF), lds, stream, z, z_stride, dh, N, F,
                       num_classes, workspace, band, dyn_N);
  }
  GEOSSL_CHECK_LAUNCH();
  hipLaunchKernelGGL(k_embedding_bwd_reduce, dim3((F + 63) / 64, num_classes), dim3(256), 0, stream, workspace, band,
                     nchunks, num_classes, F, dtable, accumulate);
  GEOSSL_CHECK_LAUNCH();
  return 0;
}

extern "C" int geossl_segment_reduce_fwd(const float* h, const int32_t* mol_ptr, int64_t B, int F, int mean, float* out,
                                         hipStream_t stream) {
  if (B <= 0) return 0;
  hipLaunchKernelGGL(k_segment_reduce_fwd, dim3((unsigned)B), dim3(F < 256 ? ((F + 63) / 64 * 64) : 256), 0, stream, h,
                     mol_ptr, (int)B, F, mean, out);
  GEOSSL_CHECK_LAUNCH();
  return 0;
}

extern "C" int geossl_segment_reduce_bwd(const float* dout, const int32_t* mol_ptr, int64_t B, int F, int mean,
                                         float* dh, int accumulate, hipStream_t stream) {
  if (B <= 0) return 0;
  hipLaunchKernelGGL(k_segment_reduce_bwd, dim3((unsigned)B), dim3(F < 256 ? ((F + 63) / 64 * 64) : 256), 0, stream,
                     dout, mol_ptr, (int)B, F, mean, dh, accumulate);
  GEOSSL_CHECK_LAUNCH();
  return 0;
}
```

### geossl_amd/csrc/tn.h

```cpp
#pragma once
#include "common.h"
#include "geossl_hip.h"

namespace geossl {

__global__ void k_reduce_partials(GeosslReduceBatch batch, const float* __restrict__ partial, int nblk, int len,
                                  int ncols, int ld, int cstride, int accumulate);

struct ReduceSeg {
  const float* partial;
  int len, ncols, ld, cstride;
  float* out[GEOSSL_TN_MAX];
};
struct ReduceMulti {
  int nseg;
  int xoff[7];
  ReduceSeg seg[6];
  ReduceMulti() : nseg(0) { xoff[0] = 0; }
  void add(const float* partial, int len, int ncols, int ld, int cstride, float* const* out, int nz) {
    ReduceSeg& g = seg[nseg];
    g.partial = partial;
    g.len = len;
    g.ncols = ncols;
    g.ld = ld;
    g.cstride = cstride;
    for (int z = 0; z < GEOSSL_TN_MAX; ++z) g.out[z] = z < nz ? out[z] : nullptr;
    xoff[nseg + 1] = xoff[nseg] + (len + 63) / 64;
    ++nseg;
  }
  int blocks() const { return xoff[nseg]; }
};
__global__ void k_reduce_multi(ReduceMulti m, int nblk, int accumulate);
__device__ __forceinline__ void reduce_multi_block(const ReduceMulti& m, int nblk, int accumulate, float (*red)[64],
                                                   int z) {
  int g = 0;
  while (g + 1 < m.nseg && (int)blockIdx.x >= m.xoff[g + 1]) ++g;
  const ReduceSeg& sg = m.seg[g];
  float* out = sg.out[z];
  if (out == nullptr) return;
  const int len = sg.len;
  const float* p = sg.partial + (size_t)z * nblk * len;
  const int lane = threadIdx.x & 63, slice = threadIdx.x >> 6;
  const int i = ((int)blockIdx.x - m.xoff[g]) * 64 + lane;
  const int per = (nblk + 3) / 4, b0 = slice * per, b1 = min(nblk, b0 + per);
  float s = 0.0f;
  if (i < len) s = kahan_sum_strided(p + i, b0, b1, len);
  red[slice][lane] = s;
  __syncthreads();
  if (slice == 0 && i < len) {
    const size_t o = (size_t)(i / sg.ncols) * sg.ld + (size_t)(i % sg.ncols) * sg.cstride;
    float v = accumulate ? out[o] : 0.0f;
    v += red[0][lane];
    v += red[1][lane];
    v += red[2][lane];
    v += red[3][lane];
    out[o] = v;
  }
}

inline int64_t tn_workspace_floats(int64_t R, int M, int N, int nprob) {
  int chunk, nblk;
  geossl_tn_plan(R, nprob, &chunk, &nblk);
  return (int64_t)nprob * nblk * ((int64_t)M * N + 2 * M);
}

}
```

### geossl_amd/csrc/wgrad.h

```cpp
#pragma once
#include "common.h"
#include "geossl_hip.h"
#include "split.h"
#include "tn.h"

namespace geossl {

struct WgradOut {
  float* dW[GEOSSL_TN_MAX];
  float* db[GEOSSL_TN_MAX];
  float* dd[GEOSSL_TN_MAX];
};

template <int NCM, int NCN, class Ops, int PIECES = 2>
__global__ __launch_bounds__(256, 2) void k_wgrad_split(Ops ops, int R, int chunk, int M, int N,
                                                        float* __restrict__ partial, float* __restrict__ partial_bias,
                                                        float* __restrict__ partial_dot,
                                                        const int32_t* __restrict__ dyn_R, int nblk, int nprob) {
  R = dyn_count(R, dyn_R);
  int z, cidx;
  if (nblk < 0) {
    nblk = (int)gridDim.x;
    z = blockIdx.y;
    cidx = blockIdx.x;
// ... 180 lines not shown
#define GEOSSL_WG_STEP(pa, pb)                                                              \
  _Pragma("unroll") for (int d = 0; d < 2; ++d) {                                           \
    if (i0 + d < TPW && wave + 4 * (i0 + d) < T)                                            \
      acc[i0 + d] = mfma_f16(af[d].pa, bf[d].pb, acc[i0 + d]);                              \
  }
        GEOSSL_WG_STEP(l, h)
        GEOSSL_WG_STEP(h, l)
        GEOSSL_WG_STEP(h, h)
#undef GEOSSL_WG_STEP
      }
    }
    }
    lds_barrier();
  };
  for (int row0 = row_begin; row0 < row_end; row0 += 32 * PF) {
#pragma unroll
    for (int p = 0; p < PF; ++p)
      if (row0 + 32 * p < row_end) tile(row0 + 32 * p, ra_[p], rb_[p]);
  }
  const size_t pb = (size_t)z * nblk + cidx;
  float* Pp = partial + pb * M * N;
#pragma unroll
  for (int i = 0; i < TPW; ++i) {
    const int t = wave + 4 * i;
    if (t >= T) continue;
    const int mb = t / NCN, nb = t % NCN, n = 32 * nb + j;
    if (n >= N) continue;
    const float kk = PIECES == 3 ? 1.0f : __builtin_amdgcn_ldexpf(1.0f, eacc[i] - 28);
#pragma unroll
    for (int r = 0; r < 16; ++r) {
      const int m = 32 * mb + c_row(r, lane);
      if (m < M) Pp[(size_t)m * N + n] = acc[i][r] * kk;
    }
  }
#pragma unroll
  for (int u = 0; u < SA; ++u) {
    const int blk = wave + 4 * u;
    if (blk >= NCM) continue;
    const float sb = bsum[u] + __shfl_xor(bsum[u], 32, 64);
    const float sd = dsum[u] + __shfl_xor(dsum[u], 32, 64);
    if (kh == 0 && 32 * blk + j < M) {
      if (partial_bias != nullptr) partial_bias[pb * M + 32 * blk + j] = sb;
      if (partial_dot != nullptr) partial_dot[pb * M + 32 * blk + j] = sd;
    }
  }
}

inline bool arith_24bit() { return getenv("GEOSSL_ARITH_24BIT") != nullptr; }

template <int NCM, int NCN, class Ops>
int launch_wgrad_split(const Ops& ops, int nprob, int64_t R, int M, int N, const WgradOut& out, int dW_ld, int dd_stride,
                       float* workspace, int accumulate, hipStream_t stream, const int32_t* dyn_R = nullptr) {
  if (nprob <= 0 || R <= 0) return 0;
  if (nprob > GEOSSL_TN_MAX) return (int)hipErrorInvalidValue;
  int chunk, nblk;
  geossl_tn_plan(R, nprob, &chunk, &nblk);
  float* partial = workspace;
  float* pbias = partial + (size_t)nprob * nblk * M * N;
  float* pdot = pbias + (size_t)nprob * nblk * M;
  bool any_b = false, any_d = false;
  for (int z = 0; z < nprob; ++z) {
    any_b |= out.db[z] != nullptr;
    any_d |= out.dd[z] != nullptr;
  }
  static const bool plain_order = getenv("GEOSSL_WGRAD_PLAIN_ORDER") != nullptr;
  const dim3 grid = plain_order ? dim3(nblk, nprob) : dim3((unsigned)(8 * ((nblk + 7) / 8) * nprob));
  const int nblk_arg = plain_order ? -1 : nblk;
  if (arith_24bit()) {
    const size_t lds = (size_t)(NCM + NCN) * 2 * 3 * 1024 + (size_t)(NCM + NCN) * sizeof(int);
    allow_big_lds(&k_wgrad_split<NCM, NCN, Ops, 3>);
    hipLaunchKernelGGL((k_wgrad_split<NCM, NCN, Ops, 3>), grid, dim3(256), lds, stream, ops, (int)R, chunk, M,
                       N, partial, any_b ? pbias : nullptr, any_d ? pdot : nullptr, dyn_R, nblk_arg, nprob);
  } else {
    const size_t lds = (size_t)(NCM + NCN) * 2 * 2 * 1024 + (size_t)(NCM + NCN) * sizeof(int);
    allow_big_lds(&k_wgrad_split<NCM, NCN, Ops>);
    hipLaunchKernelGGL((k_wgrad_split<NCM, NCN, Ops>), grid, dim3(256), lds, stream, ops, (int)R, chunk, M,
                       N, partial, any_b ? pbias : nullptr, any_d ? pdot : nullptr, dyn_R, nblk_arg, nprob);
  }
  GEOSSL_CHECK_LAUNCH();
  ReduceMulti rm;
  rm.add(partial, M * N, N, dW_ld, 1, out.dW, nprob);
  if (any_b) rm.add(pbias, M, M, M, 1, out.db, nprob);
  if (any_d) rm.add(pdot, M, M, M, dd_stride, out.dd, nprob);
  hipLaunchKernelGGL(k_reduce_multi, dim3(rm.blocks(), nprob), dim3(256), 0, stream, rm, nblk, accumulate);
  GEOSSL_CHECK_LAUNCH();
  return 0;
}

__device__ __forceinline__ void request_col8(const float* __restrict__ src, int ld, int col, int row0, int row_end,
                                             int kh, float (&v)[2][8]) {
#pragma unroll
  for (int ks = 0; ks < 2; ++ks)
#pragma unroll
    for (int e = 0; e < 8; ++e)
      v[ks][e] = __builtin_nontemporal_load(src + (size_t)min(row0 + 16 * ks + 8 * kh + e, row_end - 1) * ld + col);
}
__device__ __forceinline__ void finish_col8(int row0, int row_end, int kh, const float (&raw)[2][8],
                                            float (&out)[2][8]) {
#pragma unroll
  for (int ks = 0; ks < 2; ++ks)
#pragma unroll
    for (int e = 0; e < 8; ++e) {
      const float t = pin(raw[ks][e]);
      out[ks][e] = row0 + 16 * ks + 8 * kh + e < row_end ? t : 0.0f;
    }
}

struct PlainOps {
  GeosslTnBatch batch;
  int lda, ldb;
  static constexpr bool kDot = false;
  struct RawA { float v[2][8]; };
  struct RawB { float v[2][8]; };
  __device__ __forceinline__ void prime_a(int, int, int, int, int, RawA&) const {}
  __device__ __forceinline__ void prime_b(int, int, int, int, int, RawB&) const {}
  __device__ __forceinline__ void request_a(int z, int col, int row0, int row_end, int kh, RawA& r) const {
    request_col8(batch.A[z], lda, col, row0, row_end, kh, r.v);
  }
  __device__ __forceinline__ void request_b(int z, int col, int row0, int row_end, int kh, RawB& r) const {
    request_col8(batch.B[z], ldb, col, row0, row_end, kh, r.v);
  }
  __device__ __forceinline__ void finish_a(int, int, int row0, int row_end, int kh, RawA& r, float (&out)[2][8],
                                           float (&)[2][8]) const {
    finish_col8(row0, row_end, kh, r.v, out);
  }
  __device__ __forceinline__ void finish_b(int, int, int row0, int row_end, int kh, RawB& r, float (&out)[2][8]) const {
    finish_col8(row0, row_end, kh, r.v, out);
  }
};

}
```

### geossl_amd/ops.py

```python
import ctypes as C
import math
import os

import numpy as np
import torch
from .switches import env as _env

from . import _lib
from ._lib import call, ptr, stream
from .layout import MolLayout, get_layout

PI_F32 = float(torch.tensor(math.pi, dtype=torch.float32))
RAGGED_LOOP_MAX_MOLS = int(_env("GEOSSL_RAGGED_LOOP_MAX", 256))


def _f32(t):
    if t.dtype != torch.float32:
        raise TypeError("expected float32, got %s" % t.dtype)
    return t.contiguous()


def radius_cap(max_num_neighbors, loop=False):
    return max_num_neighbors if loop else max_num_neighbors + 1

# ... 119 lines not shown
        out += [images[i] for i in range(len(chunk))]
    return (out[:len(weights)], out[len(weights):]) if both else out


def _dyn(layout_or_dyn, field):
    d = getattr(layout_or_dyn, "dyn", layout_or_dyn)
    return None if d is None else getattr(d, field)


def linear_chain(x, stages, dyn_rows=None):
    R, F = x.shape
    assert x.stride(1) == 1 and 1 <= len(stages) <= _lib.CHAIN_MAX
    ch = _lib.Chain()
    ch.nstage = len(stages)
    outs = []
    for s, sd in enumerate(stages):
        st = ch.st[s]
        o = sd.get("out")
        if o is None and sd.get("store", True):
            o = torch.empty(R, F, dtype=torch.float32, device=x.device)
        rows_ = [a for a in (o, sd.get("res"), sd.get("tprev"), sd.get("out_act")) if a is not None]
        ld = rows_[0].stride(0) if rows_ else F
        for a in rows_:
            assert a.stride(0) == ld and a.stride(1) == 1 and a.size(0) == R and a.size(1) == F
        st.image, st.bias, st.res, st.tprev, st.out = (ptr(sd["image"]), ptr(sd.get("bias")), ptr(sd.get("res")),
                                                       ptr(sd.get("tprev")), ptr(o))
        st.out_act = ptr(sd.get("out_act"))
        st.ld, st.flags = ld, int(sd.get("flags", 0)) | (_lib.CHAIN_SAME_INPUT if sd.get("same_input") else 0)
        xin = sd.get("x")
        if xin is not None:
            assert s > 0 and xin.stride(1) == 1 and xin.size(0) == R and xin.size(1) == F
            st.xin, st.ldxin = ptr(xin), xin.stride(0)
            st.flags |= _lib.CHAIN_NEW_INPUT | (_lib.CHAIN_ADD_PREV if sd.get("add_prev") else 0)
        else:
            st.xin, st.ldxin = None, 0
        outs.append(o)
    call("geossl_linear_chain_dyn", ptr(x), x.stride(0), C.byref(ch), R, F, dyn_rows, stream())
    return outs


_LOOP_WORDS, _LOOP_STAGE0, _LOOP_STAGE_WORDS = 50, 5, 9
assert C.sizeof(_lib.LoopOp) == 8 * _LOOP_WORDS and _lib.LoopOp.chain.offset == 32 and _lib.Chain.st.offset == 8 \
    and C.sizeof(_lib.ChainStage) == 8 * _LOOP_STAGE_WORDS and _lib.ChainStage.ld.offset == 40 \
    and _lib.ChainStage.out_act.offset == 64


def layer_loop(ops_list, layout, pair_flag, N, F, stagger=0):
    plan, nblk = layout.loop_plan()
    ragged = (plan is None and F == 128 and 1 < layout.max_n <= 33 and layout.B <= RAGGED_LOOP_MAX_MOLS
              and not _env("GEOSSL_NO_RAGGED_LOOP") and len(ops_list) <= _lib.LOOP_MAX_OPS)
    if not ragged and (plan is None or F != 128 or not layout.uniform or layout.max_n > 20
                       or len(ops_list) > _lib.LOOP_MAX_OPS):
        return False
    words = [0] * (_LOOP_WORDS * len(ops_list))
    dp = lambda t_: 0 if t_ is None else t_.data_ptr()
    for i, op in enumerate(ops_list):
        b = _LOOP_WORDS * i
        if op[0] == "chain":
            _, x, stages = op
            assert x.shape == (N, F) and x.is_contiguous() and len(stages) <= 3
            words[b + 1], words[b + 4] = x.data_ptr(), len(stages)
            for s, sd in enumerate(stages):
                w = b + _LOOP_STAGE0 + _LOOP_STAGE_WORDS * s
                o, r, tp = sd.get("out"), sd.get("res"), sd.get("tprev")
                for a in (o, r, tp):
                    assert a is None or (a.shape == (N, F) and a.is_contiguous())
                words[w], words[w + 1], words[w + 2], words[w + 3], words[w + 4] = (
                    sd["image"].data_ptr(), dp(sd.get("bias")), dp(r), dp(tp), dp(o))
                words[w + 5] = F | (int(sd.get("flags", 0)) << 32)
        else:
            _, x, Wf_l, out, swap = op
            words[b], words[b + 1], words[b + 2], words[b + 3] = 1 | ((1 if swap else 0) << 32), x.data_ptr(), \
                Wf_l.data_ptr(), out.data_ptr()
    arr = np.array(words, dtype=np.uint64)
    if ragged:
        call("geossl_schnet_layer_loop_ragged", arr.ctypes.data, len(ops_list), ptr(layout.mol_ptr), ptr(layout.pair_ptr),
             ptr(pair_flag), layout.B, 1 if layout.B <= 512 else 2, N, F, stream())
        return True
    call("geossl_schnet_layer_loop", arr.ctypes.data, len(ops_list), ptr(plan), nblk, ptr(layout.mol_ptr),
         ptr(layout.pair_ptr), ptr(pair_flag), layout.max_n, 1 if layout.uniform else 0, N, F, int(stagger), stream())
    return True


def linear_wgrad(problems, R, M, N, accumulate=False, lda=None, ldb=None, ldw=None, dyn_rows=None):
    dev = problems[0][0].device
    lda, ldb, ldw = lda or M, ldb or N, ldw or N
    for lo in range(0, len(problems), _lib.TN_MAX):
        chunk = problems[lo:lo + _lib.TN_MAX]
        tb = _lib.TnBatch()
        for i, (A, Bm, dW, db) in enumerate(chunk):
            tb.A[i], tb.B[i], tb.dW[i], tb.db[i] = ptr(A), ptr(Bm), ptr(dW), ptr(db)
        nfl = _lib.load().geossl_tn_workspace_floats(R, M, N, len(chunk))
        ws = torch.empty(nfl, dtype=torch.float32, device=dev)
        call("geossl_linear_wgrad_dyn", C.byref(tb), len(chunk), R, M, N, lda, ldb, ldw, ptr(ws), 1 if accumulate else 0,
             dyn_rows, stream())


def aggregate(x, Wf_l, pair_flag, layout, swap=False, out=None, mols=None):
    N, F = x.shape
    if out is None:
        out = torch.empty_like(x)
    work = getattr(layout, "agg_work", None)
    if mols is None and work is not None and 32 < F <= 128:
        call("geossl_cfconv_aggregate_targets_dyn" if getattr(layout, "agg_targets", False)
             else "geossl_cfconv_aggregate_work_dyn", ptr(x), ptr(Wf_l), ptr(pair_flag), ptr(layout.mol_ptr),
             ptr(layout.pair_ptr), ptr(work), work.numel(), layout.max_n, F, 1 if swap else 0, ptr(out),
             _dyn(layout, "n_work"), stream())
        return out
    if getattr(layout, "dyn", None) is not None:
        raise _lib.GeosslHipError("a capacity-bucket layout needs the work-list aggregation (64 or 128 features)")
    if mols is None:
        mp, pp, order, B = ptr(layout.mol_ptr), ptr(layout.pair_ptr), layout.order, layout.B
    else:
        m0, m1, order = mols
        B = m1 - m0
        if order is not None:
            mp, pp = ptr(layout.mol_ptr), ptr(layout.pair_ptr)
        else:
            mp, pp = ptr(layout.mol_ptr) + 4 * m0, ptr(layout.pair_ptr) + 4 * m0
    call("geossl_cfconv_aggregate", ptr(x), ptr(Wf_l), ptr(pair_flag), mp, pp, ptr(order), B, layout.max_n, F,
         1 if swap else 0, ptr(out), stream())
    return out


def pair_product(a, b, layout, pair_flag, swap=False):
    N, F = a.shape
    out = torch.empty(layout.P, F, dtype=torch.float32, device=a.device)
    call("geossl_pair_product", ptr(a), ptr(b), ptr(layout.pair_i), ptr(layout.pair_j), ptr(pair_flag), layout.P, F,
         1 if swap else 0, ptr(out), stream())
    return out


def segment_reduce(h, layout, reduce):
    out = torch.empty(layout.B, h.size(1), dtype=torch.float32, device=h.device)
    call("geossl_segment_reduce_fwd", ptr(h), ptr(layout.mol_ptr), layout.B, h.size(1), 1 if reduce == "mean" else 0,
         ptr(out), stream())
    return out


def pair_distance(pos, sei0, sei1):
    pos = _f32(pos)
    S = sei0.numel()
    out = torch.empty(S, 1, dtype=torch.float32, device=pos.device)
    call("geossl_pair_distance", ptr(pos), ptr(sei0), ptr(sei1), S, ptr(out), stream())
    return out


def ddm_views(pos, noise, sei0, sei1, z=None, dyn=None):
    pos, noise = _f32(pos), _f32(noise)
    N, S = pos.size(0), sei0.numel()
    pos2 = torch.empty(2 * N, 3, dtype=torch.float32, device=pos.device)
    d01 = torch.empty(S, 1, dtype=torch.float32, device=pos.device)
    d02 = torch.empty(S, 1, dtype=torch.float32, device=pos.device)
    z2 = None
    if z is not None:
        assert z.dim() == 1 and z.dtype == torch.long and z.numel() == N
        z2 = torch.empty(2 * N, dtype=torch.long, device=pos.device)
    call("geossl_ddm_views_dyn", ptr(pos), ptr(noise), ptr(sei0), ptr(sei1), N, S, ptr(pos2), ptr(d01), ptr(d02), ptr(z),
         z.stride(0) if z is not None and N > 0 else 1, ptr(z2), _dyn(dyn, "n_atoms"), _dyn(dyn, "n_super"), stream())
    return (pos2, d01, d02) if z is None else (pos2, d01, d02, z2)


def add_scaled(a, b, alpha=1.0):
    a, b = _f32(a), _f32(b)
    out = torch.empty_like(a)
    call("geossl_axpy", ptr(a), ptr(b), float(alpha), a.numel(), ptr(out), stream())
    return out


class _RowNormalize(torch.autograd.Function):

    @staticmethod
    def forward(ctx, h, eps):
        h = _f32(h)
        N, F = h.shape
        y = torch.empty_like(h)
        norm = torch.empty(N, dtype=torch.float32, device=h.device) if ctx.needs_input_grad[0] else None
        call("geossl_row_normalize_fwd", ptr(h), N, F, float(eps), ptr(y), ptr(norm), stream())
# ... 603 lines not shown
```

### geossl_amd/pretrain_GeoSSL.py

```python
import ctypes as C
import os
import threading
import warnings
from collections import OrderedDict

import numpy as np
import torch
from .switches import env as _env

from . import _lib, ops
from ._lib import call, ptr, stream
from .layout import MolLayout

NCSN_model_01 = None
NCSN_model_02 = None


def perturb(x, positions, mu, sigma, noise=None, device_noise=False, generator=None):
    x_perturb = x
    device = positions.device
    if noise is None:
        if device_noise:
            noise = torch.empty_like(positions).normal_(mu, sigma, generator=generator)
        else:
# ... 955 lines not shown
_MT_PENDING = []


def _single_thread_backward(ticket):
    if _env("GEOSSL_KEEP_AUTOGRAD_THREADS"):
        return
    if torch.autograd.is_multithreading_enabled():
        torch.autograd.set_multithreading_enabled(False)
        token = ticket["mt_token"] = _MtToken(threading.get_ident())
        _MT_PENDING.append(token)


class _MtToken:
    __slots__ = ("thread", "live")

    def __init__(self, thread):
        self.thread, self.live = thread, True


def _restore_backward_threads(ticket=None):
    me = threading.get_ident()
    if ticket is not None:
        token = ticket.pop("mt_token", None) if isinstance(ticket, dict) else None
        todo = [] if token is None else [token]
    else:
        todo = [t for t in _MT_PENDING if t.thread == me]
    for t in todo:
        if t.live and t.thread == me:
            t.live = False
            torch.autograd.set_multithreading_enabled(True)
    _MT_PENDING[:] = [p for p in _MT_PENDING if p.live]


def _schnet_step_params(model):
    from .Geom3D.models.schnet import _core_params
    return _core_params(model)


def _autograd_step(model, n1, n2):
    eng = model.__dict__.get("_geossl_autograd_step")
    if eng is None or eng.n1 is not n1 or eng.n2 is not n2 or not eng.unchanged():
        eng = _AutogradStep(model, n1, n2)
        model.__dict__["_geossl_autograd_step"] = eng
    return eng


class DDMTrainer:

    def __init__(self, model, ncsn_01, ncsn_02, lr=5e-4, weight_decay=0.0, mu=0.0, sigma=0.3, model_3d="schnet",
                 device_noise=True, use_graph=False, overlap_heads=True, max_graphs=256, graph_mode="auto"):
        from .optim import FlatParams, FusedAdam
        from .parallel import GradAllReduce
        self.model, self.n1, self.n2 = model, ncsn_01, ncsn_02
        self.args = Args(model_3d)
        self.mu, self.sigma = mu, sigma
        self.device_noise = device_noise
        self.flat = FlatParams([model, ncsn_01, ncsn_02])
        self.opt = FusedAdam(self.flat, lr=lr, weight_decay=weight_decay)
        self.reduce = GradAllReduce(self.flat.grad)
        self.use_graph = use_graph
        self.overlap_heads = overlap_heads
        self.step_graphs = StepGraphs(self._fwd_bwd, model_3d, max_graphs, mode=graph_mode,
                                      modules=(model, ncsn_01, ncsn_02))
        self.step_graphs.zero_with_refresh = self.flat.grad
        self._zero_outside = True
        self._one = torch.ones((), dtype=torch.float32, device=self.flat.grad.device)
        self._side = None

    @property
    def _graphs(self):
        return self.step_graphs.graphs

    def _fwd_bwd(self, batch, noise):
        from . import NCSN as _ncsn
        if not (self._zero_outside and own_capture_open()):
            self.flat.zero_grad()
        if noise is None and self.device_noise:
            noise = self._draw_noise(batch)
        loss = _do_ddm_eager(self.args, batch, self.model, self.mu, self.sigma, (self.n1, self.n2), noise, True,
                             self.device_noise)
        if self._side is None and self.overlap_heads:
            self._side = torch.cuda.Stream()
        _ncsn.set_side_stream(self._side)
        try:
            with _lib.direct_grads():
                loss.backward(self._one)
        finally:
            _ncsn.set_side_stream(None)
            _ncsn.join_side_stream()
        self.flat.rebind_grads()
        return loss.detach()

    _NOISE_KEYS = _NOISE_KEYS

    def _graph_fwd_bwd(self, batch, noise):
        sg = self.step_graphs
        g = sg.lookup(batch)
        own_noise = noise is None
        if g is None:
            if not sg.capture_now(batch):
                return self._fwd_bwd(batch, noise)
            if own_noise:
                noise = self._draw_noise(batch)
            g = sg.capture(batch, noise)
            if g is None:
                self.use_graph = False
                return self._fwd_bwd(batch, noise)
            own_noise = False
        if not sg.refresh(g, batch, None if own_noise else noise):
            return self._fwd_bwd(batch, noise)
        if own_noise:
            self._draw_noise(g["batch"], into=g["noise"])
        g["graph"].replay()
        return g["loss"].clone()

    def _draw_noise(self, batch, into=None):
        if _env("GEOSSL_TORCH_DRAWS"):
            return draw_step_noise(batch, self.n1, self.n2, self.mu, self.sigma, True, None, into)
        return draw_step_noise_fused(batch, self.n1, self.n2, self.mu, self.sigma, into)

    def step(self, batch, noise=None, structure_key=None):
        if self.use_graph and ((noise is None and self.device_noise)
                               or (noise is not None and all(k in noise for k in _NOISE_KEYS))):
            loss = self._graph_fwd_bwd(batch, noise)
        else:
            loss = self._fwd_bwd(batch, noise)
        st = self.model.__dict__.get("_geossl_status")
        if st is not None:
            st.poll()
            st.arm(every=8)
        scale = self.reduce()
        self.opt.step(grad_scale=scale)
        return loss


CE_criterion = torch.nn.CrossEntropyLoss()

CONTRASTIVE_OPTIONS = ("InfoNCE", "EBM_NCE")


class ContrastiveArgs:

    def __init__(self, model_3d="schnet", normalize=False, T=0.1, num_neg=1):
        self.model_3d, self.normalize, self.T, self.num_neg = model_3d, bool(normalize), float(T), int(num_neg)


def _stock_ce(c):
    return (type(c) is torch.nn.CrossEntropyLoss and c.weight is None and c.reduction == "mean"
            and float(c.label_smoothing) == 0.0 and c.ignore_index < 0)


def _stock_bce(c):
    return c is None or (type(c) is torch.nn.BCEWithLogitsLoss and c.weight is None and c.pos_weight is None
                         and c.reduction == "mean")


def draw_views_noise(batch, mu, sigma, device_noise, given=None, into=None):
    given = given or {}
    src = given.get("pos_noise")
    if into is not None:
        t_ = into["pos_noise"]
        if src is not None:
            t_.copy_(src.view_as(t_))
        elif device_noise:
            t_.normal_(mu, sigma)
        else:
            _host_normal_into(t_, mu, sigma)
        return into
    if src is None:
# ... 186 lines not shown
```

### include/geossl_hip.h

```cpp
#ifndef GEOSSL_HIP_H
#define GEOSSL_HIP_H
#include <stdint.h>
#ifdef __HIPCC__
#include <hip/hip_runtime.h>
#else
typedef struct ihipStream_t* hipStream_t;
#endif

#ifdef __cplusplus
extern "C" {
#endif

#define GEOSSL_ABI_VERSION 1
#define GEOSSL_MAX_L 12
#define GEOSSL_TN_MAX 32
#define GEOSSL_LOSS_PARTIALS 256

#define GEOSSL_EPI_BIAS 1
#define GEOSSL_EPI_SSP 2
#define GEOSSL_EPI_RESIDUAL 4
#define GEOSSL_EPI_MUL_DSSP 8
#define GEOSSL_CHAIN_NEW_INPUT 32
#define GEOSSL_CHAIN_ADD_PREV 64
#define GEOSSL_EPI_SILU 128
// ... 266 lines not shown
                                 const int64_t* idx_i, const int64_t* inc_ptr, const int32_t* inc_idx, const float* phi,
                                 const float* fcut, const float* dir, const float* Wf, const float* bf, int64_t N, int F,
                                 int R, float* dxc, float* dmu_in, float* dWf, float* dbf, float* workspace,
                                 int accumulate, hipStream_t stream);
int geossl_painn_interaction_fwd_mma(const float* q, const float* mu, const float* xc, const int64_t* idx_j,
                                     const int32_t* row_edge, const int32_t* grp_atom, const int32_t* mol_grp,
                                     const float* phi, const float* fcut, const float* dir, const float* Wf,
                                     const float* bf, const int32_t* mol_ptr, int64_t B, int max_n, int64_t N, int F, int R,
                                     float* q_out, float* mu_out, hipStream_t stream);
int geossl_painn_interaction_fwd_mol(const float* q, const float* mu, const float* xc, const int64_t* idx_j,
                                     const int64_t* inc_ptr, const int32_t* inc_idx, const float* phi, const float* fcut,
                                     const float* dir, const float* Wf, const float* bf, const int32_t* mol_ptr,
                                     int64_t B, int max_n, int64_t N, int F, int R, float* q_out, float* mu_out,
                                     hipStream_t stream);
int64_t geossl_painn_interaction_bwd_mol_workspace_floats(int64_t N, int64_t B, int F, int R);
int geossl_painn_interaction_bwd_mol(const float* dq_out, const float* dmu_out, const float* mu, const float* xc,
                                     const int64_t* idx_i, const int64_t* inc_ptr, const int32_t* inc_idx,
                                     const float* phi, const float* fcut, const float* dir, const float* Wf,
                                     const float* bf, const int32_t* mol_ptr, int64_t B, int max_n, int64_t N, int F,
                                     int R, float* dxc, float* dmu_in, float* dWf, float* dbf, float* workspace,
                                     int accumulate, hipStream_t stream);
int geossl_painn_mix_pre_fwd(const float* q, const float* mm, int64_t N, int F, float eps, float* ctx, float* dot,
                             hipStream_t stream);
int geossl_painn_mix_post_fwd(const float* q, const float* mu, const float* mm, const float* xx, const float* dot,
                              int64_t N, int F, float* q_out, float* mu_out, hipStream_t stream);
int geossl_painn_mix_post_bwd(const float* dq_new, const float* dmu_new, const float* mm, const float* xx,
                              const float* dot, int64_t N, int F, float* dxx, float* dmm, hipStream_t stream);
int geossl_painn_mix_pre_bwd(const float* dq_new, const float* dctx, const float* ctx, const float* mm, int64_t N, int F,
                             float* dq_in, float* dmm, hipStream_t stream);
int geossl_add(const float* a, const float* b, int64_t n, float* out, hipStream_t stream);

int geossl_painn_edge_grads(const float* dq_out, const float* dmu_out, const float* mu, const float* xc,
                            const int64_t* idx_i, const int64_t* idx_j, const float* phi, const float* fcut,
                            const float* dir, const float* Wf, const float* bf, int64_t E, int F, int R, float* dphi,
                            float* dfcut, float* ddir, int accumulate, hipStream_t stream);
int geossl_painn_edge_geom_bwd(const float* pos, const int64_t* idx_i, const int64_t* idx_j, int64_t E, float cutoff,
                               const float* offsets, const float* widths, int R, const float* dphi, const float* dfcut,
                               const float* ddir, float* dr, hipStream_t stream);
int geossl_painn_position_grad(const float* dr, const int64_t* inc_i_ptr, const int32_t* inc_i_idx,
                               const int64_t* inc_j_ptr, const int32_t* inc_j_idx, int64_t N, float* dpos,
                               hipStream_t stream);

int geossl_adam_step(float* param, const float* grad, float* exp_avg, float* exp_avg_sq, int64_t n, double lr,
                     double beta1, double beta2, double eps, double weight_decay, int64_t step_count, float grad_scale,
                     hipStream_t stream);

#define GEOSSL_COPY_MAX 8
typedef struct GeosslCopyBatch {
  void* dst[GEOSSL_COPY_MAX];
  const void* src[GEOSSL_COPY_MAX];
  int64_t bytes[GEOSSL_COPY_MAX];
} GeosslCopyBatch;
int geossl_copy_n(const GeosslCopyBatch* batch, int n, hipStream_t stream);
int geossl_ddm_views_dyn(const float* pos, const float* noise, const int64_t* sei0, const int64_t* sei1, int64_t N,
                         int64_t S, float* pos2, float* d01, float* d02, const int64_t* z, int64_t z_stride, int64_t* z2,
                         const int32_t* dyn_N, const int32_t* dyn_S, hipStream_t stream);
int geossl_embedding_fwd_dyn(const int64_t* z, int64_t z_stride, const float* table, int num_classes, int64_t N, int F,
                             float* out, int32_t* status, const int32_t* dyn_N, hipStream_t stream);
int geossl_embedding_bwd_dyn(const int64_t* z, int64_t z_stride, const float* dh, int num_classes, int64_t N, int F,
                             float* dtable, float* workspace, int accumulate, const int32_t* dyn_N, hipStream_t stream);
int geossl_cfconv_filter_fwd_dyn(const float* pair_d, const float* pair_c, int64_t P, const GeosslFilterWeights* w, int L,
                                 int F, int G, const float* offset, float coeff, float* T, float* Wf,
                                 const int32_t* dyn_P, hipStream_t stream);
int geossl_cfconv_filter_bwd_dyn(const float* pair_d, const float* pair_c, const uint8_t* pair_flag,
                                 const int32_t* pair_i, const int32_t* pair_j, int64_t P, int64_t N,
                                 const GeosslFilterWeights* w, const GeosslFilterGradIn* g, int L, int F, int G,
                                 const float* offset, float coeff, const float* T, const GeosslFilterGradOut* out,
                                 float* workspace, int accumulate, const int32_t* dyn_P, const int32_t* dyn_N,
                                 hipStream_t stream);
int geossl_cfconv_aggregate_work_dyn(const float* x, const float* Wf, const uint8_t* pair_flag, const int32_t* mol_ptr,
                                     const int32_t* pair_ptr, const int32_t* work, int64_t nwork, int max_n, int F,
                                     int swap, float* out, const int32_t* dyn_nwork, hipStream_t stream);
int geossl_linear_chain_dyn(const float* X, int ldx, const GeosslChain* chain, int64_t R, int F, const int32_t* dyn_R,
                            hipStream_t stream);
int geossl_linear_wgrad_dyn(const GeosslTnBatch* batch, int nprob, int64_t R, int M, int N, int lda, int ldb, int ldw,
                            float* workspace, int accumulate, const int32_t* dyn_R, hipStream_t stream);
int geossl_ddm_loss_fwd2_dyn(const GeosslNcsnHeadFwd* heads, const int64_t* batch, const int64_t* sei0,
                             const int64_t* sei1, int64_t S, int F, const int32_t* dyn_S, const int32_t* dyn_view,
                             hipStream_t stream);
int geossl_ddm_loss_bwd_fused2_dyn(const GeosslNcsnHeadBwd* heads, const int64_t* sei0, const int64_t* sei1, int64_t S,
                                   int64_t N, int F, const int64_t* stats_divisor, const float* gout,
                                   const int64_t* inc_ptr, const int32_t* inc_idx, int accumulate, const int32_t* dyn_S,
                                   const int32_t* dyn_view, hipStream_t stream);

int64_t geossl_painn_group_capacity(int64_t E2, int64_t N2);
int geossl_painn_edge_layout(const int64_t* src_i, const int64_t* src_j, int64_t E, const int32_t* mol_ptr, int64_t N,
                             int64_t B, int64_t N2cap, int64_t* idx_i2, int64_t* idx_j2, int64_t* iptr_i,
                             int32_t* ilist_i, int64_t* iptr_j, int32_t* ilist_j, int32_t* row_edge, int32_t* grp_atom,
                             int32_t* mol_grp, int32_t* mol_grp_end, int32_t* status, hipStream_t stream);
int geossl_painn_edge_geom_dyn(const float* pos, const int64_t* idx_i, const int64_t* idx_j, int64_t E, float cutoff,
                               const float* offsets, const float* widths, int R, float* dir, float* fcut, float* phi,
                               const int32_t* dyn_E, hipStream_t stream);
int geossl_painn_interaction_fwd_mma_dyn(const float* q, const float* mu, const float* xc, const int64_t* idx_j,
                                         const int32_t* row_edge, const int32_t* grp_atom, const int32_t* mol_grp,
                                         const float* phi, const float* fcut, const float* dir, const float* Wf,
                                         const float* bf, const int32_t* mol_ptr, int64_t B, int max_n, int64_t N, int F,
                                         int R, float* q_out, float* mu_out, const int32_t* mol_grp_end,
                                         hipStream_t stream);
int geossl_painn_stage_cap(int kind, int F, int R);
int geossl_painn_interaction_fwd_atoms(const float* q, const float* mu, const float* xc, const int64_t* idx_j,
                                       const int64_t* inc_ptr, const int32_t* inc_idx, const float* phi,
                                       const float* fcut, const float* dir, const float* Wf, const float* bf,
                                       const int32_t* atom_list, int64_t nlist, const int32_t* dyn_nlist, int F, int R,
                                       float* q_out, float* mu_out, hipStream_t stream);
int geossl_painn_interaction_bwd_atoms(const float* dq_out, const float* dmu_out, const float* mu, const float* xc,
                                       const int64_t* idx_i, const int64_t* inc_ptr, const int32_t* inc_idx,
                                       const float* phi, const float* fcut, const float* dir, const float* Wf,
                                       const float* bf, const int32_t* atom_list, int64_t nlist,
                                       const int32_t* dyn_nlist, int F, int R, float* dxc, float* dmu_in, float* dWf,
                                       float* dbf, float* workspace, int accumulate, hipStream_t stream);
int geossl_painn_interaction_bwd_mol_skip(const float* dq_out, const float* dmu_out, const float* mu, const float* xc,
                                          const int64_t* idx_i, const int64_t* inc_ptr, const int32_t* inc_idx,
                                          const float* phi, const float* fcut, const float* dir, const float* Wf,
                                          const float* bf, const int32_t* mol_ptr, int64_t B, int max_n, int64_t N, int F,
                                          int R, float* dxc, float* dmu_in, float* dWf, float* dbf, float* workspace,
                                          int accumulate, hipStream_t stream);
int geossl_painn_mix_pre_fwd_dyn(const float* q, const float* mm, int64_t N, int F, float eps, float* ctx, float* dot,
                                 const int32_t* dyn_N, hipStream_t stream);
int geossl_painn_mix_post_fwd_dyn(const float* q, const float* mu, const float* mm, const float* xx, const float* dot,
                                  int64_t N, int F, float* q_out, float* mu_out, const int32_t* dyn_N,
                                  hipStream_t stream);
int geossl_painn_mix_post_bwd_dyn(const float* dq_new, const float* dmu_new, const float* mm, const float* xx,
                                  const float* dot, int64_t N, int F, float* dxx, float* dmm, const int32_t* dyn_N,
                                  hipStream_t stream);
int geossl_painn_mix_pre_bwd_dyn(const float* dq_new, const float* dctx, const float* ctx, const float* mm, int64_t N,
                                 int F, float* dq_in, float* dmm, const int32_t* dyn_N, hipStream_t stream);

int geossl_tape_unary(int kind, const float* x, int64_t n, float alpha, float beta, float* y, hipStream_t stream);
int geossl_tape_binary(int op, const float* a, int amode, const float* b, int bmode, int64_t R, int D, float scale,
                       float* y, hipStream_t stream);
int64_t geossl_tape_colsum_workspace_floats(int64_t R, int D);
int geossl_tape_reduce(int kind, const float* x, int64_t R, int D, float* y, float* workspace, hipStream_t stream);
int geossl_tape_gather_rows(const float* src, const void* idx, int idx64, int64_t E, int D, float* out,
                            hipStream_t stream);
int geossl_tape_scatter_rows(const float* src, const void* ptr, int ptr64, const int32_t* perm, int64_t N, int D,
                             float* out, hipStream_t stream);
int geossl_tape_copy2d(const float* src, int64_t ld_src, float* dst, int64_t ld_dst, int64_t R, int C,
                       hipStream_t stream);
int geossl_tape_fill(float* dst, int64_t n, float value, hipStream_t stream);

typedef struct GeosslGather {
  const int64_t* x_src;
  const float* pos_src;
  const int32_t* src_off;
  const int32_t* mol_ptr;
  int64_t* x_dst;
  float* pos_dst;
  int64_t* batch_dst;
  const int32_t* se_ptr;
  int64_t* sei0;
  int64_t* sei1;
  const int32_t* pair_ptr2;
  int32_t* pair_i;
  int32_t* pair_j;
  const int64_t* inc_ptr;
  int32_t* inc_idx;
  const int64_t* e0_src;
  const int64_t* e1_src;
  const int32_t* e_src_off;
  const int32_t* e_ptr;
  int64_t* e0_dst;
  int64_t* e1_dst;
  float* zero;
  int64_t zero_count;
  int32_t x_cols;
  int32_t option;
// ... 141 lines not shown
```

Measured before the change: 385,700.

## Defer backward partial-sum reductions into a single end-of-step glue kernel

Adds a deferral mechanism so the separate reduce kernels that finish weight gradients (linear wgrad, embedding bwd, cfconv filter bwd, NCSN heads) are queued while backward runs. All of them are then executed in one batched reduction launch when backward completes. The aim is to cut per-kernel launch overhead and tail latency from many small reduce kernels. In exchange, the partial workspaces must be kept alive until the flush, more global state and locking are introduced, and gradients are not final until the flush runs.

```diff
diff --git a/geossl_amd/Geom3D/models/schnet.py b/geossl_amd/Geom3D/models/schnet.py
--- a/geossl_amd/Geom3D/models/schnet.py
+++ b/geossl_amd/Geom3D/models/schnet.py
@@ -314,21 +314,24 @@
             fw.w1[l], fw.b1[l], fw.w2[l], fw.b2[l] = ptr(lp[0]), ptr(lp[1]), ptr(lp[2]), ptr(lp[3])
             gin.x[l], gin.dagg[l] = ptr(sv["xs"][l]), ptr(daggs[l])
         if want_params:
-            ops.linear_wgrad(probs, N, F, F, accumulate=bool(accum), dyn_rows=dN2)
+            _lib.glue_need_direct(direct)
+            ops.linear_wgrad(probs, N, F, F, accumulate=bool(accum), dyn_rows=dN2, defer=True)
             nfl = _lib.load().geossl_embedding_bwd_workspace_floats(emb_w.size(0), F)
             ws = torch.empty(nfl, dtype=torch.float32, device=dev)
             z = ctx.z
-            call("geossl_embedding_bwd_dyn", ptr(z), z.stride(0) if z.numel() else 1, ptr(dh), emb_w.size(0), N, F,
-                 ptr(g_emb), ptr(ws), accum, dN2, st)
+            with _lib.glue_scope(ws):
+                call("geossl_embedding_bwd_dyn", ptr(z), z.stride(0) if z.numel() else 1, ptr(dh), emb_w.size(0), N, F,
+                     ptr(g_emb), ptr(ws), accum, dN2, st)
             if P > 0:
                 gout = _lib.FilterGradOut()
                 for l, gl in enumerate(g_layers):
                     gout.dw1[l], gout.db1[l], gout.dw2[l], gout.db2[l] = ptr(gl[0]), ptr(gl[1]), ptr(gl[2]), ptr(gl[3])
                 nfl = _lib.load().geossl_cfconv_filter_bwd_workspace_floats(P, L, F, G)
                 ws2 = torch.empty(nfl, dtype=torch.float32, device=dev)
-                call("geossl_cfconv_filter_bwd_dyn", ptr(sv["pair_d"]), ptr(sv["pair_c"]), ptr(sv["pair_flag"]),
-                     ptr(lay.pair_i), ptr(lay.pair_j), P, N, C.byref(fw), C.byref(gin), L, F, G, ptr(cfg["offset"]),
-                     cfg["coeff"], ptr(sv["T"]), C.byref(gout), ptr(ws2), accum, dP2, dN2, st)
+                with _lib.glue_scope(ws2):
+                    call("geossl_cfconv_filter_bwd_dyn", ptr(sv["pair_d"]), ptr(sv["pair_c"]), ptr(sv["pair_flag"]),
+                         ptr(lay.pair_i), ptr(lay.pair_j), P, N, C.byref(fw), C.byref(gin), L, F, G, ptr(cfg["offset"]),
+                         cfg["coeff"], ptr(sv["T"]), C.byref(gout), ptr(ws2), accum, dP2, dN2, st)
             elif not direct:
                 for gl in g_layers:
                     for k in range(4):
diff --git a/geossl_amd/NCSN.py b/geossl_amd/NCSN.py
--- a/geossl_amd/NCSN.py
+++ b/geossl_amd/NCSN.py
@@ -254,9 +254,11 @@
                 ptr(hs[k]), ctx.out_scale, ptr(dfeat), ptr(demb), ptr(grow), ptr(ws1), ptr(dh))
             keep += [dfeat, demb, grow, ws1]
             dhs.append(dh)
-        call("geossl_ddm_loss_bwd_fused2_dyn", C.byref(heads), ptr(sel.sei0), ptr(sel.sei1), S, sel.N if dyn is not None else N,
-             Fd, ptr(sel.stats), ptr(gout), ptr(sel.inc_ptr), ptr(sel.inc_idx), 1 if direct else 0,
-             None if dyn is None else dyn.n_super, None if dyn is None else dyn.n_atoms, st)
+        _lib.glue_need_direct(direct)
+        with _lib.glue_scope(*keep[3::4]):
+            call("geossl_ddm_loss_bwd_fused2_dyn", C.byref(heads), ptr(sel.sei0), ptr(sel.sei1), S,
+                 sel.N if dyn is not None else N, Fd, ptr(sel.stats), ptr(gout), ptr(sel.inc_ptr), ptr(sel.inc_idx),
+                 1 if direct else 0, None if dyn is None else dyn.n_super, None if dyn is None else dyn.n_atoms, st)
         head = ((dh_all, None) if dyn is not None else (dhs[0], dhs[1])) + (None,) * 11
         if direct:
             return head + (None,) * len(grads)
diff --git a/geossl_amd/_lib.py b/geossl_amd/_lib.py
--- a/geossl_amd/_lib.py
+++ b/geossl_amd/_lib.py
@@ -280,6 +280,13 @@
                                           vp]),
     "geossl_triple_angles": (i32, [vp, i64, vp, vp, vp, i64, vp, vp]),
     "geossl_gather_triples": (i32, [vp, i64, vp, vp, vp, vp, i64, vp, vp, vp, vp, vp]),
+    "geossl_step_defer_begin": (i32, [vp, i32]),
+    "geossl_step_defer_arm": (i32, [i32]),
+    "geossl_step_defer_cancel": (i32, []),
+    "geossl_step_defer_pending": (i32, []),
+    "geossl_step_defer_describe": (i32, [i32, vp]),
+    "geossl_step_reduce": (i32, [vp]),
+    "geossl_reduce_partials_deferred": (i32, [vp, i32, vp, i32, i32, i32, i32, i32, i32, vp]),
 }
 
 _lib = None
@@ -351,6 +358,63 @@
         for p in params)
 
 
+_GLUE = {"open": False, "keep": []}
+
+
+def glue_wanted():
+    from .switches import env
+    return not env("GEOSSL_STEP_SEPARATE_GLUE")
+
+
+def glue_begin():
+    call("geossl_step_defer_begin", stream(), 0)
+    _GLUE["open"] = True
+    del _GLUE["keep"][:]
+
+
+def glue_active():
+    return _GLUE["open"]
+
+
+class glue_scope:
+
+    def __init__(self, *tensors):
+        self.tensors = tensors
+
+    def __enter__(self):
+        self.on = _GLUE["open"]
+        if self.on:
+            _GLUE["keep"].extend(t for t in self.tensors if t is not None)
+            load().geossl_step_defer_arm(1)
+        return self
+
+    def __exit__(self, *exc):
+        if self.on:
+            load().geossl_step_defer_arm(0)
+        return False
+
+
+def glue_flush():
+    if not _GLUE["open"]:
+        return
+    _GLUE["open"] = False
+    try:
+        call("geossl_step_reduce", stream())
+    finally:
+        del _GLUE["keep"][:]
+
+
+def glue_cancel():
+    _GLUE["open"] = False
+    del _GLUE["keep"][:]
+    load().geossl_step_defer_cancel()
+
+
+def glue_need_direct(direct):
+    if not direct:
+        glue_flush()
+
+
 class StatusWord:
 
     def __init__(self, device, message):
diff --git a/geossl_amd/build.py b/geossl_amd/build.py
--- a/geossl_amd/build.py
+++ b/geossl_amd/build.py
@@ -15,7 +15,8 @@
 
 SOURCE_FLAGS = {"painn_mma.hip": ["-fno-slp-vectorize"], "distance_head.hip": ["-fno-slp-vectorize"],
                 "charge_head.hip": ["-fno-slp-vectorize"], "infograph_head.hip": ["-fno-slp-vectorize"],
-                "property_head.hip": ["-fno-slp-vectorize"], "torsion_head.hip": ["-fno-slp-vectorize"]}
+                "property_head.hip": ["-fno-slp-vectorize"], "torsion_head.hip": ["-fno-slp-vectorize"],
+                "step_glue.hip": ["-fno-slp-vectorize"]}
 
 
 def _headers():
diff --git a/geossl_amd/csrc/common.h b/geossl_amd/csrc/common.h
--- a/geossl_amd/csrc/common.h
+++ b/geossl_amd/csrc/common.h
@@ -127,6 +127,25 @@
   }
   return s;
 }
+template <int U>
+__device__ __forceinline__ float kahan_sum_strided_batched(const float* __restrict__ p, int b0, int b1, int stride) {
+#pragma clang fp reassociate(off) contract(off)
+  float s = 0.0f, c = 0.0f;
+  for (int b = b0; b < b1; b += U) {
+    float v[U];
+#pragma unroll
+    for (int u = 0; u < U; ++u) v[u] = p[(size_t)min(b + u, b1 - 1) * stride];
+#pragma unroll
+    for (int u = 0; u < U; ++u)
+      if (b + u < b1) {
+        const float y = v[u] - c;
+        const float t = s + y;
+        c = (t - s) - y;
+        s = t;
+      }
+  }
+  return s;
+}
 
 __device__ __forceinline__ int dyn_count(int cap, const int32_t* __restrict__ dyn) {
   return dyn != nullptr ? min(cap, *dyn) : cap;
diff --git a/geossl_amd/csrc/filter_bwd.hip b/geossl_amd/csrc/filter_bwd.hip
--- a/geossl_amd/csrc/filter_bwd.hip
+++ b/geossl_amd/csrc/filter_bwd.hip
@@ -1149,6 +1149,9 @@
   rm.add(pb1, F, F, F, 1, out->db1, L);
   rm.add(pw2, F * F, F, F, 1, out->dw2, L);
   rm.add(pb2, F, F, F, 1, out->db2, L);
+  const int deferred = glue_defer_multi(rm, L, nb, accumulate, stream);
+  if (deferred < 0) return (int)hipErrorInvalidValue;
+  if (deferred) return 0;
   hipLaunchKernelGGL(k_reduce_multi, dim3(rm.blocks(), L), dim3(256), 0, stream, rm, nb, accumulate);
   GEOSSL_CHECK_LAUNCH();
   return 0;
diff --git a/geossl_amd/csrc/ncsn_bwd.hip b/geossl_amd/csrc/ncsn_bwd.hip
--- a/geossl_amd/csrc/ncsn_bwd.hip
+++ b/geossl_amd/csrc/ncsn_bwd.hip
@@ -2,6 +2,7 @@
 #include "geossl_hip.h"
 #include "split.h"
 #include "tn.h"
+#include "step_glue.h"
 
 using namespace geossl;
 
@@ -641,22 +642,8 @@
     reduce_multi_block(m, nblk, accumulate, red, 0);
     return;
   }
-  const int H = F / 2, len = H + 3 * F + 2;
-  const int i = ((int)blockIdx.x - mb) * 4 + (int)(threadIdx.x >> 6), lane = threadIdx.x & 63;
-  if (i >= len) return;
-  float s = 0.0f;
-  for (int b = lane; b < nblk; b += 64) s += psm[(size_t)b * len + i];
-  s = wave_sum(s);
-  if (lane == 0) {
-    float* dst;
-    if (i < H) dst = g.o3_w + i;
-    else if (i < H + F) dst = g.in_w2 + (i - H);
-    else if (i < H + 2 * F) dst = g.in_w1 + (i - H - F);
-    else if (i < H + 3 * F) dst = g.in_b1 + (i - H - 2 * F);
-    else if (i == H + 3 * F) dst = g.o3_b;
-    else dst = g.in_b2;
-    *dst = accumulate ? *dst + s : s;
-  }
+  ncsn_small_reduce_block(psm, nblk, F, accumulate, g.o3_w, g.in_w2, g.in_w1, g.in_b1, g.o3_b, g.in_b2,
+                          (int)blockIdx.x - mb);
 }
 __global__ __launch_bounds__(256) void k_ncsn_reduce_all(ReduceMulti m, int nblk, int accumulate,
                                                          const float* __restrict__ psm, int F, GeosslNcsnGrads g) {
@@ -793,9 +780,17 @@
     rm[k].add(a[k].pw2, H * F, F, F, 1, o2w, 1);
     rm[k].add(a[k].pb2, H, H, H, 1, o2b, 1);
   }
-  hipLaunchKernelGGL(k_ncsn_reduce_all2, dim3(rm[0].blocks() + (H + 3 * F + 2 + 3) / 4, 2), dim3(256), 0, stream, rm[0],
-                     rm[1], nb, accumulate, a[0].psm, a[1].psm, F, heads[0].grads, heads[1].grads);
-  GEOSSL_CHECK_LAUNCH();
+  const int deferred = glue_defer_multi(rm[0], 1, nb, accumulate, stream);
+  if (deferred < 0) return (int)hipErrorInvalidValue;
+  if (deferred && (glue_defer_ncsn_small(a[0].psm, nb, F, accumulate, heads[0].grads, stream) != 1 ||
+                   glue_defer_multi(rm[1], 1, nb, accumulate, stream) != 1 ||
+                   glue_defer_ncsn_small(a[1].psm, nb, F, accumulate, heads[1].grads, stream) != 1))
+    return (int)hipErrorInvalidValue;
+  if (!deferred) {
+    hipLaunchKernelGGL(k_ncsn_reduce_all2, dim3(rm[0].blocks() + (H + 3 * F + 2 + 3) / 4, 2), dim3(256), 0, stream, rm[0],
+                       rm[1], nb, accumulate, a[0].psm, a[1].psm, F, heads[0].grads, heads[1].grads);
+    GEOSSL_CHECK_LAUNCH();
+  }
   if (heads[0].dh != nullptr && heads[1].dh != nullptr)
     return launch_incidence_gather2(heads[0].dfeat, heads[1].dfeat, inc_ptr, inc_idx, N, F, heads[0].dh, heads[1].dh, stream,
                                     dyn_view);
diff --git a/geossl_amd/csrc/schnet.hip b/geossl_amd/csrc/schnet.hip
--- a/geossl_amd/csrc/schnet.hip
+++ b/geossl_amd/csrc/schnet.hip
@@ -2,6 +2,7 @@
 #include "aggregate_reg.h"
 #include "geossl_hip.h"
 #include "tn.h"
+#include "step_glue.h"
 
 #include <cstdlib>
 
@@ -304,7 +305,6 @@
   }
 }
 
-#define GEOSSL_EMB_CHUNKS 512
 template <int NG>
 __global__ void k_embedding_bwd_partial(const int64_t* __restrict__ z, int64_t zs, const float* __restrict__ dh,
                                         int64_t N, int F, int C, float* __restrict__ partial, int2* __restrict__ band,
@@ -359,47 +359,10 @@
 __global__ __launch_bounds__(256) void k_embedding_bwd_reduce(const float* __restrict__ partial,
                                                               const int2* __restrict__ band, int nchunks, int C, int F,
                                                               float* __restrict__ dtable, int accumulate) {
-  constexpr int PERMAX = GEOSSL_EMB_CHUNKS / 4;
-  static_assert(PERMAX == 128, "two chunks per lane");
-  const int PER = nchunks / 4;
   __shared__ float red[4][64];
-  __shared__ int hits[4][PERMAX];
-  const int c = blockIdx.y, lane = threadIdx.x & 63, slice = threadIdx.x >> 6;
-  const int f = blockIdx.x * 64 + lane;
-  int n = 0;
-#pragma unroll
-  for (int h = 0; h < 2; ++h) {
-    const int b = slice * PER + 64 * h + lane;
-    const int2 r = 64 * h + lane < PER ? band[b] : make_int2(1, 0);
-    const bool hit = c >= r.x && c <= r.y;
-    const unsigned long long m = __ballot(hit);
-    if (hit) hits[slice][n + __popcll(m & ((1ull << lane) - 1ull))] = b;
-    n += __popcll(m);
-  }
-  __builtin_amdgcn_wave_barrier();
-  float s = 0.0f;
-  if (f < F) {
-#pragma clang fp reassociate(off) contract(off)
-    float k = 0.0f;
-    const float* p = partial + (size_t)c * F + f;
-#pragma unroll 4
-    for (int i = 0; i < n; ++i) {
-      const float y = p[(size_t)hits[slice][i] * C * F] - k;
-      const float t = s + y;
-      k = (t - s) - y;
-      s = t;
-    }
-  }
-  red[slice][lane] = s;
-  __syncthreads();
-  if (slice == 0 && f < F) {
-    float v = accumulate ? dtable[(size_t)c * F + f] : 0.0f;
-    v += red[0][lane];
-    v += red[1][lane];
-    v += red[2][lane];
-    v += red[3][lane];
-    dtable[(size_t)c * F + f] = v;
-  }
+  __shared__ int hits[4][GEOSSL_EMB_CHUNKS / 4];
+  embedding_bwd_reduce_block(partial, band, nchunks, C, F, dtable, accumulate, (int)blockIdx.y, (int)blockIdx.x, red,
+                             hits);
 }
 __global__ void k_segment_reduce_fwd(const float* __restrict__ h, const int32_t* __restrict__ mol_ptr, int B, int F,
                                      int mean, float* __restrict__ out) {
@@ -643,6 +606,9 @@
                        num_classes, workspace, band, dyn_N);
   }
   GEOSSL_CHECK_LAUNCH();
+  const int deferred = glue_defer_embedding(workspace, band, nchunks, num_classes, F, dtable, accumulate, stream);
+  if (deferred < 0) return (int)hipErrorInvalidValue;
+  if (deferred) return 0;
   hipLaunchKernelGGL(k_embedding_bwd_reduce, dim3((F + 63) / 64, num_classes), dim3(256), 0, stream, workspace, band,
                      nchunks, num_classes, F, dtable, accumulate);
   GEOSSL_CHECK_LAUNCH();
diff --git a/geossl_amd/csrc/step_glue.h b/geossl_amd/csrc/step_glue.h
--- /dev/null
+++ b/geossl_amd/csrc/step_glue.h
@@ -0,0 +1,96 @@
+#pragma once
+#include "tn.h"
+
+#define GEOSSL_EMB_CHUNKS 512
+
+namespace geossl {
+
+template <int U = 4>
+__device__ __forceinline__ void embedding_bwd_reduce_block(const float* __restrict__ partial,
+                                                           const int2* __restrict__ band, int nchunks, int C, int F,
+                                                           float* __restrict__ dtable, int accumulate, int c, int xb,
+                                                           float (*red)[64], int (*hits)[GEOSSL_EMB_CHUNKS / 4]) {
+  constexpr int PERMAX = GEOSSL_EMB_CHUNKS / 4;
+  static_assert(PERMAX == 128, "two chunks per lane");
+  const int PER = nchunks / 4;
+  const int lane = threadIdx.x & 63, slice = threadIdx.x >> 6;
+  const int f = xb * 64 + lane;
+  int n = 0;
+#pragma unroll
+  for (int h = 0; h < 2; ++h) {
+    const int b = slice * PER + 64 * h + lane;
+    const int2 r = 64 * h + lane < PER ? band[b] : make_int2(1, 0);
+    const bool hit = c >= r.x && c <= r.y;
+    const unsigned long long m = __ballot(hit);
+    if (hit) hits[slice][n + __popcll(m & ((1ull << lane) - 1ull))] = b;
+    n += __popcll(m);
+  }
+  __builtin_amdgcn_wave_barrier();
+  float s = 0.0f;
+  if (f < F) {
+#pragma clang fp reassociate(off) contract(off)
+    float k = 0.0f;
+    const float* p = partial + (size_t)c * F + f;
+    if (U > 4) {
+      for (int i = 0; i < n; i += U) {
+        float v[U];
+#pragma unroll
+        for (int u = 0; u < U; ++u) v[u] = p[(size_t)hits[slice][min(i + u, n - 1)] * C * F];
+#pragma unroll
+        for (int u = 0; u < U; ++u)
+          if (i + u < n) {
+            const float y = v[u] - k;
+            const float t = s + y;
+            k = (t - s) - y;
+            s = t;
+          }
+      }
+    } else {
+#pragma unroll 4
+      for (int i = 0; i < n; ++i) {
+        const float y = p[(size_t)hits[slice][i] * C * F] - k;
+        const float t = s + y;
+        k = (t - s) - y;
+        s = t;
+      }
+    }
+  }
+  red[slice][lane] = s;
+  __syncthreads();
+  if (slice == 0 && f < F) {
+    float v = accumulate ? dtable[(size_t)c * F + f] : 0.0f;
+    v += red[0][lane];
+    v += red[1][lane];
+    v += red[2][lane];
+    v += red[3][lane];
+    dtable[(size_t)c * F + f] = v;
+  }
+}
+
+__device__ __forceinline__ void ncsn_small_reduce_block(const float* __restrict__ psm, int nblk, int F, int accumulate,
+                                                        float* o3_w, float* in_w2, float* in_w1, float* in_b1,
+                                                        float* o3_b, float* in_b2, int vb) {
+  const int H = F / 2, len = H + 3 * F + 2;
+  const int i = vb * 4 + (int)(threadIdx.x >> 6), lane = threadIdx.x & 63;
+  if (i >= len) return;
+  float s = 0.0f;
+  for (int b = lane; b < nblk; b += 64) s += psm[(size_t)b * len + i];
+  s = wave_sum(s);
+  if (lane == 0) {
+    float* dst;
+    if (i < H) dst = o3_w + i;
+    else if (i < H + F) dst = in_w2 + (i - H);
+    else if (i < H + 2 * F) dst = in_w1 + (i - H - F);
+    else if (i < H + 3 * F) dst = in_b1 + (i - H - 2 * F);
+    else if (i == H + 3 * F) dst = o3_b;
+    else dst = in_b2;
+    *dst = accumulate ? *dst + s : s;
+  }
+}
+
+int glue_defer_embedding(const float* partial, const int2* band, int nchunks, int C, int F, float* dtable,
+                         int accumulate, hipStream_t stream);
+int glue_defer_ncsn_small(const float* psm, int nblk, int F, int accumulate, const GeosslNcsnGrads& g,
+                          hipStream_t stream);
+
+}
diff --git a/geossl_amd/csrc/step_glue.hip b/geossl_amd/csrc/step_glue.hip
--- /dev/null
+++ b/geossl_amd/csrc/step_glue.hip
@@ -0,0 +1,322 @@
+#include "common.h"
+#include "geossl_hip.h"
+#include "step_glue.h"
+#include "tn.h"
+
+#include <algorithm>
+#include <mutex>
+#include <vector>
+
+using namespace geossl;
+
+namespace {
+
+enum { GLUE_MULTI = 1, GLUE_EMBEDDING = 2, GLUE_NCSN_SMALL = 3 };
+#define GLUE_MAX_ITEMS 8
+#define GLUE_MAX_SEGS 24
+#define GLUE_MAX_OUTS 160
+#define GLUE_BATCH 16
+
+struct GlueSeg {
+  const float* partial;
+  int len, ncols, ld, cstride;
+  int x0;
+  int out0;
+};
+struct GlueItem {
+  int kind, nblk, accumulate, nz;
+  int seg0, nseg, xblocks, F;
+  int C, nchunks, pad0, pad1;
+  const float* p0;
+  const int2* band;
+  float* dst[6];
+};
+struct StepReduceArgs {
+  int nitems;
+  int boff[GLUE_MAX_ITEMS + 1];
+  GlueItem item[GLUE_MAX_ITEMS];
+  GlueSeg seg[GLUE_MAX_SEGS];
+  float* out[GLUE_MAX_OUTS];
+};
+static_assert(sizeof(StepReduceArgs) <= 3584, "the table is a kernel argument (4 KB with the implicit ones)");
+
+__global__ __launch_bounds__(256) void k_step_reduce(StepReduceArgs a) {
+  __shared__ float red[4][64];
+  __shared__ int hits[4][GEOSSL_EMB_CHUNKS / 4];
+  const int block = (int)blockIdx.x;
+  int it = 0;
+  while (it + 1 < a.nitems && block >= a.boff[it + 1]) ++it;
+  const GlueItem& im = a.item[it];
+  const int vb = block - a.boff[it];
+  if (im.kind == GLUE_MULTI) {
+    const int z = vb / im.xblocks, xb = vb - z * im.xblocks;
+    int g = im.seg0;
+    while (g + 1 < im.seg0 + im.nseg && xb >= a.seg[g + 1].x0) ++g;
+    const GlueSeg& sg = a.seg[g];
+    float* out = a.out[sg.out0 + z];
+    if (out == nullptr) return;
+    reduce_seg_block<GLUE_BATCH>(sg.partial + (size_t)z * im.nblk * sg.len, sg.len, sg.ncols, sg.ld, sg.cstride, out, im.nblk,
+                     im.accumulate, xb - sg.x0, red);
+  } else if (im.kind == GLUE_EMBEDDING) {
+    const int c = vb / im.xblocks, xb = vb - c * im.xblocks;
+    embedding_bwd_reduce_block<GLUE_BATCH>(im.p0, im.band, im.nchunks, im.C, im.F, im.dst[0], im.accumulate, c, xb, red, hits);
+  } else {
+    ncsn_small_reduce_block(im.p0, im.nblk, im.F, im.accumulate, im.dst[0], im.dst[1], im.dst[2], im.dst[3], im.dst[4],
+                            im.dst[5], vb);
+  }
+}
+
+struct Region {
+  uintptr_t lo, hi;
+};
+inline bool overlaps(const std::vector<Region>& a, const std::vector<Region>& b) {
+  for (const Region& x : a)
+    for (const Region& y : b)
+      if (x.lo < y.hi && y.lo < x.hi) return true;
+  return false;
+}
+inline Region region(const void* p, size_t bytes) {
+  const uintptr_t lo = reinterpret_cast<uintptr_t>(p);
+  return Region{lo, lo + bytes};
+}
+
+struct Glue {
+  std::mutex mu;
+  bool open = false, armed = false, dry = false;
+  hipStream_t stream = nullptr;
+  StepReduceArgs args;
+  int nseg = 0, nout = 0, flushes = 0;
+  std::vector<Region> parts, outs;
+  void clear() {
+    args.nitems = 0;
+    args.boff[0] = 0;
+    nseg = nout = 0;
+    parts.clear();
+    outs.clear();
+  }
+};
+Glue& glue() {
+  static Glue g;
+  return g;
+}
+
+int flush_locked(Glue& g) {
+  if (g.args.nitems == 0) return 0;
+  const int blocks = g.args.boff[g.args.nitems];
+  ++g.flushes;
+  int rc = 0;
+  if (!g.dry && blocks > 0) {
+    hipLaunchKernelGGL(k_step_reduce, dim3(blocks), dim3(256), 0, g.stream, g.args);
+    rc = (int)hipGetLastError();
+  }
+  g.clear();
+  return rc;
+}
+
+int admit_locked(Glue& g, hipStream_t stream, int nseg, int nout, const std::vector<Region>& parts,
+                 const std::vector<Region>& outs) {
+  if (!g.open || !g.armed || stream != g.stream) return 0;
+  if (nseg > GLUE_MAX_SEGS || nout > GLUE_MAX_OUTS) return 0;
+  if (overlaps(parts, g.parts) || overlaps(parts, g.outs) || overlaps(outs, g.parts)) return -1;
+  if (overlaps(outs, g.outs) || g.args.nitems == GLUE_MAX_ITEMS || g.nseg + nseg > GLUE_MAX_SEGS ||
+      g.nout + nout > GLUE_MAX_OUTS) {
+    if (flush_locked(g) != 0) return -2;
+  }
+  return 1;
+}
+void commit_locked(Glue& g, const GlueItem& im, int blocks, const std::vector<Region>& parts,
+                   const std::vector<Region>& outs) {
+  const int i = g.args.nitems++;
+  g.args.item[i] = im;
+  g.args.boff[i + 1] = g.args.boff[i] + blocks;
+  g.parts.insert(g.parts.end(), parts.begin(), parts.end());
+  g.outs.insert(g.outs.end(), outs.begin(), outs.end());
+}
+
+}
+
+namespace geossl {
+
+int glue_defer_multi(const ReduceMulti& m, int nz, int nblk, int accumulate, hipStream_t stream) {
+  Glue& g = glue();
+  std::lock_guard<std::mutex> lock(g.mu);
+  if (!g.open || !g.armed || stream != g.stream) return 0;
+  if (m.nseg <= 0 || nz <= 0 || nz > GEOSSL_TN_MAX || nblk <= 0) return 0;
+  std::vector<Region> parts, outs;
+  for (int s = 0; s < m.nseg; ++s) {
+    const ReduceSeg& sg = m.seg[s];
+    if (sg.len <= 0 || sg.ncols <= 0) return 0;
+    parts.push_back(region(sg.partial, (size_t)nz * nblk * sg.len * sizeof(float)));
+    const size_t span = (size_t)((sg.len - 1) / sg.ncols) * sg.ld + (size_t)(std::min(sg.len, sg.ncols) - 1) * sg.cstride + 1;
+    for (int z = 0; z < nz; ++z)
+      if (sg.out[z] != nullptr) outs.push_back(region(sg.out[z], span * sizeof(float)));
+  }
+  const int ok = admit_locked(g, stream, m.nseg, m.nseg * nz, parts, outs);
+  if (ok <= 0) return ok;
+  GlueItem im = {};
+  im.kind = GLUE_MULTI;
+  im.nblk = nblk;
+  im.accumulate = accumulate;
+  im.nz = nz;
+  im.seg0 = g.nseg;
+  im.nseg = m.nseg;
+  im.xblocks = m.blocks();
+  for (int s = 0; s < m.nseg; ++s) {
+    const ReduceSeg& sg = m.seg[s];
+    GlueSeg& d = g.args.seg[g.nseg++];
+    d.partial = sg.partial;
+    d.len = sg.len;
+    d.ncols = sg.ncols;
+    d.ld = sg.ld;
+    d.cstride = sg.cstride;
+    d.x0 = m.xoff[s];
+    d.out0 = g.nout;
+    for (int z = 0; z < nz; ++z) g.args.out[g.nout++] = sg.out[z];
+  }
+  commit_locked(g, im, im.xblocks * nz, parts, outs);
+  return 1;
+}
+
+int glue_defer_embedding(const float* partial, const int2* band, int nchunks, int C, int F, float* dtable,
+                         int accumulate, hipStream_t stream) {
+  Glue& g = glue();
+  std::lock_guard<std::mutex> lock(g.mu);
+  if (!g.open || !g.armed || stream != g.stream) return 0;
+  std::vector<Region> parts = {region(partial, (size_t)nchunks * C * F * sizeof(float)),
+                               region(band, (size_t)nchunks * sizeof(int2))};
+  std::vector<Region> outs = {region(dtable, (size_t)C * F * sizeof(float))};
+  const int ok = admit_locked(g, stream, 0, 0, parts, outs);
+  if (ok <= 0) return ok;
+  GlueItem im = {};
+  im.kind = GLUE_EMBEDDING;
+  im.accumulate = accumulate;
+  im.xblocks = (F + 63) / 64;
+  im.F = F;
+  im.C = C;
+  im.nchunks = nchunks;
+  im.p0 = partial;
+  im.band = band;
+  im.dst[0] = dtable;
+  commit_locked(g, im, im.xblocks * C, parts, outs);
+  return 1;
+}
+
+int glue_defer_ncsn_small(const float* psm, int nblk, int F, int accumulate, const GeosslNcsnGrads& gr,
+                          hipStream_t stream) {
+  Glue& g = glue();
+  std::lock_guard<std::mutex> lock(g.mu);
+  if (!g.open || !g.armed || stream != g.stream) return 0;
+  const int H = F / 2, len = H + 3 * F + 2;
+  std::vector<Region> parts = {region(psm, (size_t)nblk * len * sizeof(float))};
+  std::vector<Region> outs = {region(gr.o3_w, H * sizeof(float)),  region(gr.in_w2, F * sizeof(float)),
+                              region(gr.in_w1, F * sizeof(float)), region(gr.in_b1, F * sizeof(float)),
+                              region(gr.o3_b, sizeof(float)),      region(gr.in_b2, sizeof(float))};
+  const int ok = admit_locked(g, stream, 0, 0, parts, outs);
+  if (ok <= 0) return ok;
+  GlueItem im = {};
+  im.kind = GLUE_NCSN_SMALL;
+  im.nblk = nblk;
+  im.accumulate = accumulate;
+  im.F = F;
+  im.p0 = psm;
+  im.dst[0] = gr.o3_w;
+  im.dst[1] = gr.in_w2;
+  im.dst[2] = gr.in_w1;
+  im.dst[3] = gr.in_b1;
+  im.dst[4] = gr.o3_b;
+  im.dst[5] = gr.in_b2;
+  commit_locked(g, im, (len + 3) / 4, parts, outs);
+  return 1;
+}
+
+}
+
+extern "C" int geossl_step_defer_begin(hipStream_t stream, int dry_run) {
+  Glue& g = glue();
+  std::lock_guard<std::mutex> lock(g.mu);
+  g.clear();
+  g.open = true;
+  g.armed = false;
+  g.dry = dry_run != 0;
+  g.stream = stream;
+  g.flushes = 0;
+  return 0;
+}
+
+extern "C" int geossl_step_defer_cancel(void) {
+  Glue& g = glue();
+  std::lock_guard<std::mutex> lock(g.mu);
+  g.clear();
+  g.open = g.armed = false;
+  return 0;
+}
+
+extern "C" int geossl_step_defer_arm(int on) {
+  Glue& g = glue();
+  std::lock_guard<std::mutex> lock(g.mu);
+  g.armed = g.open && on != 0;
+  return 0;
+}
+
+extern "C" int geossl_step_defer_pending(void) {
+  Glue& g = glue();
+  std::lock_guard<std::mutex> lock(g.mu);
+  return g.open ? g.args.nitems : -1;
+}
+
+extern "C" int geossl_step_defer_describe(int i, int64_t* out) {
+  Glue& g = glue();
+  std::lock_guard<std::mutex> lock(g.mu);
+  if (out == nullptr || !g.open) return (int)hipErrorInvalidValue;
+  if (i < 0) {
+    out[0] = g.args.nitems;
+    out[1] = g.nseg;
+    out[2] = g.nout;
+    out[3] = g.args.boff[g.args.nitems];
+    out[4] = g.flushes;
+    out[5] = g.dry ? 1 : 0;
+    out[6] = (int64_t)g.parts.size();
+    out[7] = (int64_t)g.outs.size();
+    return 0;
+  }
+  if (i >= g.args.nitems) return (int)hipErrorInvalidValue;
+  const GlueItem& im = g.args.item[i];
+  out[0] = im.kind;
+  out[1] = g.args.boff[i];
+  out[2] = g.args.boff[i + 1] - g.args.boff[i];
+  out[3] = im.nblk;
+  out[4] = im.kind == GLUE_MULTI ? im.nz : 1;
+  out[5] = im.accumulate;
+  out[6] = (int64_t)reinterpret_cast<uintptr_t>(im.kind == GLUE_MULTI ? g.args.seg[im.seg0].partial : im.p0);
+  out[7] = (int64_t)reinterpret_cast<uintptr_t>(im.kind == GLUE_MULTI ? g.args.out[g.args.seg[im.seg0].out0] : im.dst[0]);
+  return 0;
+}
+
+extern "C" int geossl_step_reduce(hipStream_t stream) {
+  Glue& g = glue();
+  std::lock_guard<std::mutex> lock(g.mu);
+  if (!g.open) return 0;
+  if (stream != g.stream) return (int)hipErrorInvalidValue;
+  const int rc = flush_locked(g);
+  g.open = g.armed = false;
+  return rc;
+}
+
+extern "C" int geossl_reduce_partials_deferred(const GeosslReduceBatch* batch, int nz, const float* partial, int nblk,
+                                               int len, int ncols, int ld, int cstride, int accumulate,
+                                               hipStream_t stream) {
+  if (batch == nullptr || nz <= 0 || nz > GEOSSL_TN_MAX || nblk <= 0 || len <= 0 || ncols <= 0) return (int)hipErrorInvalidValue;
+  ReduceMulti rm;
+  rm.add(partial, len, ncols, ld, cstride, batch->out, nz);
+  const int deferred = glue_defer_multi(rm, nz, nblk, accumulate, stream);
+  if (deferred < 0) return (int)hipErrorInvalidValue;
+  if (deferred) return 0;
+  {
+    Glue& g = glue();
+    std::lock_guard<std::mutex> lock(g.mu);
+    if (g.open && g.dry) return 0;
+  }
+  hipLaunchKernelGGL(k_reduce_multi, dim3(rm.blocks(), nz), dim3(256), 0, stream, rm, nblk, accumulate);
+  GEOSSL_CHECK_LAUNCH();
+  return 0;
+}
diff --git a/geossl_amd/csrc/tn.h b/geossl_amd/csrc/tn.h
--- a/geossl_amd/csrc/tn.h
+++ b/geossl_amd/csrc/tn.h
@@ -31,24 +31,19 @@
   int blocks() const { return xoff[nseg]; }
 };
 __global__ void k_reduce_multi(ReduceMulti m, int nblk, int accumulate);
-__device__ __forceinline__ void reduce_multi_block(const ReduceMulti& m, int nblk, int accumulate, float (*red)[64],
-                                                   int z) {
-  int g = 0;
-  while (g + 1 < m.nseg && (int)blockIdx.x >= m.xoff[g + 1]) ++g;
-  const ReduceSeg& sg = m.seg[g];
-  float* out = sg.out[z];
-  if (out == nullptr) return;
-  const int len = sg.len;
-  const float* p = sg.partial + (size_t)z * nblk * len;
+template <int U = 4>
+__device__ __forceinline__ void reduce_seg_block(const float* __restrict__ p, int len, int ncols, int ld, int cstride,
+                                                 float* __restrict__ out, int nblk, int accumulate, int xb,
+                                                 float (*red)[64]) {
   const int lane = threadIdx.x & 63, slice = threadIdx.x >> 6;
-  const int i = ((int)blockIdx.x - m.xoff[g]) * 64 + lane;
+  const int i = xb * 64 + lane;
   const int per = (nblk + 3) / 4, b0 = slice * per, b1 = min(nblk, b0 + per);
   float s = 0.0f;
-  if (i < len) s = kahan_sum_strided(p + i, b0, b1, len);
+  if (i < len) s = (U > 4 ? kahan_sum_strided_batched<U>(p + i, b0, b1, len) : kahan_sum_strided(p + i, b0, b1, len));
   red[slice][lane] = s;
   __syncthreads();
   if (slice == 0 && i < len) {
-    const size_t o = (size_t)(i / sg.ncols) * sg.ld + (size_t)(i % sg.ncols) * sg.cstride;
+    const size_t o = (size_t)(i / ncols) * ld + (size_t)(i % ncols) * cstride;
     float v = accumulate ? out[o] : 0.0f;
     v += red[0][lane];
     v += red[1][lane];
@@ -57,6 +52,22 @@
     out[o] = v;
   }
 }
+__device__ __forceinline__ void reduce_multi_block(const ReduceMulti& m, int nblk, int accumulate, float (*red)[64],
+                                                   int z, int xb) {
+  int g = 0;
+  while (g + 1 < m.nseg && xb >= m.xoff[g + 1]) ++g;
+  const ReduceSeg& sg = m.seg[g];
+  float* out = sg.out[z];
+  if (out == nullptr) return;
+  reduce_seg_block(sg.partial + (size_t)z * nblk * sg.len, sg.len, sg.ncols, sg.ld, sg.cstride, out, nblk, accumulate,
+                   xb - m.xoff[g], red);
+}
+__device__ __forceinline__ void reduce_multi_block(const ReduceMulti& m, int nblk, int accumulate, float (*red)[64],
+                                                   int z) {
+  reduce_multi_block(m, nblk, accumulate, red, z, (int)blockIdx.x);
+}
+
+int glue_defer_multi(const ReduceMulti& m, int nz, int nblk, int accumulate, hipStream_t stream);
 
 inline int64_t tn_workspace_floats(int64_t R, int M, int N, int nprob) {
   int chunk, nblk;
diff --git a/geossl_amd/csrc/wgrad.h b/geossl_amd/csrc/wgrad.h
--- a/geossl_amd/csrc/wgrad.h
+++ b/geossl_amd/csrc/wgrad.h
@@ -286,6 +286,9 @@
   rm.add(partial, M * N, N, dW_ld, 1, out.dW, nprob);
   if (any_b) rm.add(pbias, M, M, M, 1, out.db, nprob);
   if (any_d) rm.add(pdot, M, M, M, dd_stride, out.dd, nprob);
+  const int deferred = glue_defer_multi(rm, nprob, nblk, accumulate, stream);
+  if (deferred < 0) return (int)hipErrorInvalidValue;
+  if (deferred) return 0;
   hipLaunchKernelGGL(k_reduce_multi, dim3(rm.blocks(), nprob), dim3(256), 0, stream, rm, nblk, accumulate);
   GEOSSL_CHECK_LAUNCH();
   return 0;
diff --git a/geossl_amd/ops.py b/geossl_amd/ops.py
--- a/geossl_amd/ops.py
+++ b/geossl_amd/ops.py
@@ -225,7 +225,18 @@
     return True
 
 
-def linear_wgrad(problems, R, M, N, accumulate=False, lda=None, ldb=None, ldw=None, dyn_rows=None):
+class _NoScope:
+    def __enter__(self):
+        return self
+
+    def __exit__(self, *exc):
+        return False
+
+
+_NO_SCOPE = _NoScope()
+
+
+def linear_wgrad(problems, R, M, N, accumulate=False, lda=None, ldb=None, ldw=None, dyn_rows=None, defer=False):
     dev = problems[0][0].device
     lda, ldb, ldw = lda or M, ldb or N, ldw or N
     for lo in range(0, len(problems), _lib.TN_MAX):
@@ -235,8 +246,9 @@
             tb.A[i], tb.B[i], tb.dW[i], tb.db[i] = ptr(A), ptr(Bm), ptr(dW), ptr(db)
         nfl = _lib.load().geossl_tn_workspace_floats(R, M, N, len(chunk))
         ws = torch.empty(nfl, dtype=torch.float32, device=dev)
-        call("geossl_linear_wgrad_dyn", C.byref(tb), len(chunk), R, M, N, lda, ldb, ldw, ptr(ws), 1 if accumulate else 0,
-             dyn_rows, stream())
+        with _lib.glue_scope(ws) if defer else _NO_SCOPE:
+            call("geossl_linear_wgrad_dyn", C.byref(tb), len(chunk), R, M, N, lda, ldb, ldw, ptr(ws),
+                 1 if accumulate else 0, dyn_rows, stream())
 
 
 def aggregate(x, Wf_l, pair_flag, layout, swap=False, out=None, mols=None):
diff --git a/geossl_amd/pretrain_GeoSSL.py b/geossl_amd/pretrain_GeoSSL.py
--- a/geossl_amd/pretrain_GeoSSL.py
+++ b/geossl_amd/pretrain_GeoSSL.py
@@ -1061,9 +1061,18 @@
         if self._side is None and self.overlap_heads:
             self._side = torch.cuda.Stream()
         _ncsn.set_side_stream(self._side)
+        glue = self.args.model_3d == "schnet" and _lib.glue_wanted()
         try:
+            if glue:
+                _lib.glue_begin()
             with _lib.direct_grads():
                 loss.backward(self._one)
+            if glue:
+                _lib.glue_flush()
+        except BaseException:
+            if glue:
+                _lib.glue_cancel()
+            raise
         finally:
             _ncsn.set_side_stream(None)
             _ncsn.join_side_stream()
diff --git a/include/geossl_hip.h b/include/geossl_hip.h
--- a/include/geossl_hip.h
+++ b/include/geossl_hip.h
@@ -372,6 +372,15 @@
                                    int64_t N, int F, const int64_t* stats_divisor, const float* gout,
                                    const int64_t* inc_ptr, const int32_t* inc_idx, int accumulate, const int32_t* dyn_S,
                                    const int32_t* dyn_view, hipStream_t stream);
+
+int geossl_step_defer_begin(hipStream_t stream, int dry_run);
+int geossl_step_defer_arm(int on);
+int geossl_step_defer_cancel(void);
+int geossl_step_defer_pending(void);
+int geossl_step_defer_describe(int i, int64_t* out);
+int geossl_step_reduce(hipStream_t stream);
+int geossl_reduce_partials_deferred(const GeosslReduceBatch* batch, int nz, const float* partial, int nblk, int len,
+                                    int ncols, int ld, int cstride, int accumulate, hipStream_t stream);
 
 int64_t geossl_painn_group_capacity(int64_t E2, int64_t N2);
 int geossl_painn_edge_layout(const int64_t* src_i, const int64_t* src_j, int64_t E, const int32_t* mol_ptr, int64_t N,
```

Result: no change. 387,200, median of 6 (+0.4%).
